# yisol/IDM-VTON

Measured on AMD Instinct MI355X. Metric: try-on images/sec at 768x1024, 30 DDIM steps, guidance 2.0, higher is better.
Workload: dtype bf16; 1 GPU; BASELINE.json configs[1]: 768x1024, 30 steps, batch 2/GPU, guidance 2.0, bf16 storage / fp32 accumulate, scheduler ddim, hipGraph on, GarmentNet batched over 6 timesteps, GarmentNet(block b+1)||TryonNet(block b) two-stream overlap on; images_per_call=2, parallelism=dp1 (image shards, one start-up RCCL weight broadcast), rccl_ranks=1

## Files before the change

### idm-vton_amd/csrc/elementwise.hip

```cpp
#include "common.cuh"
#include <string.h>

static thread_local char g_err[512] = "";
int idmvton_set_error(int code, const char* fmt, ...) {
    va_list ap; va_start(ap, fmt); vsnprintf(g_err, sizeof(g_err), fmt, ap); va_end(ap);
    return code;
}
extern "C" const char* idmvton_last_error(void) { return g_err; }
extern "C" int idmvton_abi_version(void) { return 9; }

template <typename T>
__global__ void pack_input_kernel(const idmvton_pack_input_args a) {
    const int idx = blockIdx.x * blockDim.x + threadIdx.x;
    const int total = 2 * a.B * a.hw;
    if (idx >= total) return;
    const int b2 = idx / a.hw, pix = idx - b2 * a.hw;
    const int b = b2 % a.B;
    T* o = (T*)a.out + (size_t)idx * a.cpad;
    const T* cond = (const T*)a.cond + (size_t)idx * 9;
#pragma unroll
    for (int c = 0; c < 4; ++c) o[c] = (T)a.latents[((size_t)b * 4 + c) * a.hw + pix];
#pragma unroll
    for (int c = 0; c < 9; ++c) o[4 + c] = cond[c];
    for (int c = 13; c < a.cpad; ++c) o[c] = (T)0.f;
}
extern "C" int idmvton_pack_input(const idmvton_pack_input_args* a, void* stream) {
    CHECK_ARG(a && a->latents && a->cond && a->out, IDMVTON_E_ARG, "pack_input: null pointer");
    CHECK_ARG(a->dtype == IDMVTON_F16 || a->dtype == IDMVTON_BF16, IDMVTON_E_DTYPE, "pack_input: dtype %d", a->dtype);
    CHECK_ARG(a->B > 0 && a->hw > 0 && a->cpad >= 13, IDMVTON_E_SHAPE, "pack_input: B=%d hw=%d cpad=%d", a->B, a->hw, a->cpad);
    const int total = 2 * a->B * a->hw;
    const dim3 grid((total + 255) / 256), block(256);
    if (a->dtype == IDMVTON_BF16) hipLaunchKernelGGL((pack_input_kernel<bf16_t>), grid, block, 0, (hipStream_t)stream, *a);
    else hipLaunchKernelGGL((pack_input_kernel<f16_t>), grid, block, 0, (hipStream_t)stream, *a);
    CHECK_LAUNCH("pack_input");
    return IDMVTON_OK;
}

template <typename T>
__global__ void cfg_step_kernel(const idmvton_cfg_step_args a) {
    const int idx = blockIdx.x * blockDim.x + threadIdx.x;
    if (idx >= a.B * a.hw) return;
    const int b = idx / a.hw, pix = idx - b * a.hw;
    const float c_x = a.coef[0], c_eps = a.coef[1], sigma = a.coef[2], g = a.coef[3];
    const T* eu = (const T*)a.eps_nhwc + ((size_t)b * a.hw + pix) * a.ldc;
    const T* ec = (const T*)a.eps_nhwc + ((size_t)(a.B + b) * a.hw + pix) * a.ldc;
#pragma unroll
    for (int c = 0; c < 4; ++c) {
        const size_t o = ((size_t)b * 4 + c) * a.hw + pix;
        const float u = (float)eu[c], t = (float)ec[c];
        const float eps = u + g * (t - u);
        float x = c_x * a.latents[o] + c_eps * eps;
        if (a.noise) x += sigma * a.noise[o];
        a.latents[o] = x;
    }
}
extern "C" int idmvton_cfg_step(const idmvton_cfg_step_args* a, void* stream) {
    CHECK_ARG(a && a->eps_nhwc && a->latents && a->coef, IDMVTON_E_ARG, "cfg_step: null pointer");
    CHECK_ARG(a->dtype == IDMVTON_F16 || a->dtype == IDMVTON_BF16, IDMVTON_E_DTYPE, "cfg_step: dtype %d", a->dtype);
    CHECK_ARG(a->B > 0 && a->hw > 0 && a->ldc >= 4, IDMVTON_E_SHAPE, "cfg_step: B=%d hw=%d ldc=%d", a->B, a->hw, a->ldc);
    const dim3 grid((a->B * a->hw + 255) / 256), block(256);
    if (a->dtype == IDMVTON_BF16) hipLaunchKernelGGL((cfg_step_kernel<bf16_t>), grid, block, 0, (hipStream_t)stream, *a);
    else hipLaunchKernelGGL((cfg_step_kernel<f16_t>), grid, block, 0, (hipStream_t)stream, *a);
    CHECK_LAUNCH("cfg_step");
    return IDMVTON_OK;
}

template <typename T>
__global__ void layout_kernel(const idmvton_layout_args a) {
    const size_t idx = (size_t)blockIdx.x * blockDim.x + threadIdx.x;
    if (idx >= (size_t)a.B * a.HW) return;
    const int b = (int)(idx / a.HW), pix = (int)(idx - (size_t)b * a.HW);
    if (a.to_nhwc) {
        const float* s = (const float*)a.src;
        if (a.flags & IDMVTON_LAYOUT_SPLIT) {
            T* d = (T*)a.dst + idx * 2 * a.cpad;
            for (int c = 0; c < a.C; ++c) {
                const float f = s[((size_t)b * a.C + c) * a.HW + pix] * a.scale + a.shift;
                const T hi = (T)f;
                d[c] = hi; d[a.cpad + c] = (T)(f - (float)hi);
            }
            for (int c = a.C; c < a.cpad; ++c) { d[c] = (T)0.f; d[a.cpad + c] = (T)0.f; }
            return;
        }
        T* d = (T*)a.dst + idx * a.cpad;
        for (int c = 0; c < a.C; ++c) d[c] = (T)(s[((size_t)b * a.C + c) * a.HW + pix] * a.scale + a.shift);
        for (int c = a.C; c < a.cpad; ++c) d[c] = (T)0.f;
    } else {
        float* d = (float*)a.dst;
        if (a.flags & IDMVTON_LAYOUT_NHWC_F32) {
            const float* s = (const float*)a.src + idx * a.cpad;
            for (int c = 0; c < a.C; ++c) d[((size_t)b * a.C + c) * a.HW + pix] = s[c] * a.scale + a.shift;
            return;
        }
        const T* s = (const T*)a.src + idx * a.cpad;
        for (int c = 0; c < a.C; ++c) d[((size_t)b * a.C + c) * a.HW + pix] = (float)s[c] * a.scale + a.shift;
    }
}
extern "C" int idmvton_layout(const idmvton_layout_args* a, void* stream) {
    CHECK_ARG(a && a->src && a->dst, IDMVTON_E_ARG, "layout: null pointer");
    CHECK_ARG(a->dtype == IDMVTON_F16 || a->dtype == IDMVTON_BF16, IDMVTON_E_DTYPE, "layout: dtype %d", a->dtype);
    CHECK_ARG(a->B > 0 && a->C > 0 && a->HW > 0 && a->cpad >= a->C, IDMVTON_E_SHAPE, "layout: B=%d C=%d HW=%d cpad=%d", a->B, a->C, a->HW, a->cpad);
    CHECK_ARG((a->flags & ~3) == 0 && !((a->flags & IDMVTON_LAYOUT_SPLIT) && !a->to_nhwc) && !((a->flags & IDMVTON_LAYOUT_NHWC_F32) && a->to_nhwc),
              IDMVTON_E_ARG, "layout: flags=%d (SPLIT goes with to_nhwc, NHWC_F32 with the reverse)", a->flags);
    const size_t total = (size_t)a->B * a->HW;
    const dim3 grid((unsigned)((total + 255) / 256)), block(256);
    if (a->dtype == IDMVTON_BF16) hipLaunchKernelGGL((layout_kernel<bf16_t>), grid, block, 0, (hipStream_t)stream, *a);
    else hipLaunchKernelGGL((layout_kernel<f16_t>), grid, block, 0, (hipStream_t)stream, *a);
    CHECK_LAUNCH("layout");
    return IDMVTON_OK;
}

template <typename T>
__global__ __launch_bounds__(256) void split_rows_kernel(const idmvton_split_args a) {
    typedef typename VT<T>::v8 v8;
    const int nchunk = a.cols >> 3;
    const size_t idx = (size_t)blockIdx.x * 256 + threadIdx.x;
    if (idx >= (size_t)a.rows * nchunk) return;
    const int row = (int)(idx / nchunk), c = (int)(idx - (size_t)row * nchunk) * 8;
    const float4* p = (const float4*)(a.src + (size_t)row * a.lds + c);
    const float4 t0 = p[0], t1 = p[1];
    const float v[8] = {t0.x, t0.y, t0.z, t0.w, t1.x, t1.y, t1.z, t1.w};
    v8 hi, lo;
#pragma unroll
    for (int j = 0; j < 8; ++j) { hi[j] = (T)v[j]; lo[j] = (T)(v[j] - (float)hi[j]); }
    T* d = (T*)a.dst + (size_t)row * a.ldd + c;
    *(v8*)d = hi;
    if (a.mode == IDMVTON_SPLIT_ACT) *(v8*)(d + a.cols) = lo;
    else { *(v8*)(d + a.cols) = hi; *(v8*)(d + 2 * a.cols) = lo; }
}
template <typename T>
__global__ __launch_bounds__(256) void split_t_kernel(const idmvton_split_args a) {
    typedef typename VT<T>::v8 v8;
    __shared__ float tile[64][65];
    const int r0 = blockIdx.y * 64, c0 = blockIdx.x * 64;
    for (int i = threadIdx.x; i < 64 * 64; i += 256) {
        const int r = i >> 6, c = i & 63;
        tile[r][c] = (r0 + r < a.rows && c0 + c < a.cols) ? a.src[(size_t)(r0 + r) * a.lds + c0 + c] : 0.f;
    }
    __syncthreads();
    for (int i = threadIdx.x; i < 64 * 8; i += 256) {
        const int c = i >> 3, rc = (i & 7) * 8;
        if (c0 + c >= a.cols || r0 + rc >= a.rows) continue;
        v8 hi, lo;
#pragma unroll
        for (int j = 0; j < 8; ++j) { const float f = tile[rc + j][c]; hi[j] = (T)f; lo[j] = (T)(f - (float)hi[j]); }
        T* d = (T*)a.dst + (size_t)(c0 + c) * a.ldd + r0 + rc;
        *(v8*)d = hi; *(v8*)(d + a.rows) = hi; *(v8*)(d + 2 * a.rows) = lo;
    }
}
extern "C" int idmvton_split(const idmvton_split_args* a, void* stream) {
    CHECK_ARG(a && a->src && a->dst, IDMVTON_E_ARG, "split: null pointer");
    CHECK_ARG(a->dtype == IDMVTON_F16 || a->dtype == IDMVTON_BF16, IDMVTON_E_DTYPE, "split: dtype %d", a->dtype);
    CHECK_ARG(a->mode >= IDMVTON_SPLIT_ACT && a->mode <= IDMVTON_SPLIT_W3T, IDMVTON_E_ARG, "split: mode %d", a->mode);
    CHECK_ARG(a->rows > 0 && a->cols > 0 && a->lds >= a->cols, IDMVTON_E_SHAPE, "split: rows=%d cols=%d lds=%d", a->rows, a->cols, a->lds);
    CHECK_ARG(((uintptr_t)a->dst & 15) == 0 && a->ldd % 8 == 0, IDMVTON_E_ALIGN, "split: dst alignment / ldd=%d", a->ldd);
    hipStream_t st = (hipStream_t)stream;
    if (a->mode == IDMVTON_SPLIT_W3T) {
        CHECK_ARG(a->rows % 8 == 0 && a->ldd >= 3 * a->rows, IDMVTON_E_SHAPE, "split: W3T needs rows %% 8 == 0 and ldd >= 3 rows (rows=%d ldd=%d)", a->rows, a->ldd);
        const dim3 grid((a->cols + 63) / 64, (a->rows + 63) / 64), block(256);
        if (a->dtype == IDMVTON_BF16) hipLaunchKernelGGL((split_t_kernel<bf16_t>), grid, block, 0, st, *a);
        else hipLaunchKernelGGL((split_t_kernel<f16_t>), grid, block, 0, st, *a);
    } else {
        const int k = a->mode == IDMVTON_SPLIT_ACT ? 2 : 3;
        CHECK_ARG(a->cols % 8 == 0 && a->lds % 4 == 0 && ((uintptr_t)a->src & 15) == 0 && a->ldd >= k * a->cols, IDMVTON_E_SHAPE,
                  "split: cols=%d lds=%d ldd=%d (cols %% 8 == 0, lds %% 4 == 0, ldd >= %d cols)", a->cols, a->lds, a->ldd, k);
        const size_t total = (size_t)a->rows * (a->cols >> 3);
        const dim3 grid((unsigned)((total + 255) / 256)), block(256);
        if (a->dtype == IDMVTON_BF16) hipLaunchKernelGGL((split_rows_kernel<bf16_t>), grid, block, 0, st, *a);
        else hipLaunchKernelGGL((split_rows_kernel<f16_t>), grid, block, 0, st, *a);
    }
    CHECK_LAUNCH("split");
    return IDMVTON_OK;
}

template <typename T>
__global__ void vae_sample_kernel(const idmvton_vae_sample_args a) {
    const int idx = blockIdx.x * blockDim.x + threadIdx.x;
    if (idx >= a.B * a.hw) return;
    const int b = idx / a.hw, pix = idx - b * a.hw;
    const T* m = (const T*)a.moments + (size_t)idx * a.ldm;
#pragma unroll
    for (int c = 0; c < 4; ++c) {
        const size_t o = ((size_t)b * 4 + c) * a.hw + pix;
        const float mean = (float)m[c];
        const float lv = fminf(fmaxf((float)m[4 + c], -30.f), 20.f);
        a.z[o] = (mean + __expf(0.5f * lv) * a.noise[o]) * a.scale;
    }
}
extern "C" int idmvton_vae_sample(const idmvton_vae_sample_args* a, void* stream) {
    CHECK_ARG(a && a->moments && a->noise && a->z, IDMVTON_E_ARG, "vae_sample: null pointer");
    CHECK_ARG(a->dtype == IDMVTON_F16 || a->dtype == IDMVTON_BF16, IDMVTON_E_DTYPE, "vae_sample: dtype %d", a->dtype);
    CHECK_ARG(a->B > 0 && a->hw > 0 && a->ldm >= 8, IDMVTON_E_SHAPE, "vae_sample: B=%d hw=%d ldm=%d", a->B, a->hw, a->ldm);
    const dim3 grid((a->B * a->hw + 255) / 256), block(256);
    if (a->dtype == IDMVTON_BF16) hipLaunchKernelGGL((vae_sample_kernel<bf16_t>), grid, block, 0, (hipStream_t)stream, *a);
    else hipLaunchKernelGGL((vae_sample_kernel<f16_t>), grid, block, 0, (hipStream_t)stream, *a);
    CHECK_LAUNCH("vae_sample");
    return IDMVTON_OK;
}

typedef __attribute__((ext_vector_type(8))) int i32x8;
__global__ void probe_mfma_kernel(int which, const void* a, const void* b, float* c) {
    const int lane = threadIdx.x;
    f32x16 acc;
#pragma unroll
    for (int r = 0; r < 16; ++r) acc[r] = 0.f;
    if (which == 0) acc = VT<bf16_t>::mfma(((const bf16x8*)a)[lane], ((const bf16x8*)b)[lane], acc);
    else if (which == 2) acc = __builtin_amdgcn_mfma_scale_f32_32x32x64_f8f6f4(((const i32x8*)a)[lane], ((const i32x8*)b)[lane], acc, 0, 0, 0, 0x7f7f7f7f, 0, 0x7f7f7f7f);
    else if (which == 3) acc = __builtin_amdgcn_mfma_scale_f32_32x32x64_f8f6f4(((const i32x8*)a)[lane], ((const i32x8*)b)[lane], acc, 0, 0, 0, 0x7c7c7c7c, 0, (int)0x80808080);
    else acc = VT<f16_t>::mfma(((const f16x8*)a)[lane], ((const f16x8*)b)[lane], acc);
#pragma unroll
    for (int r = 0; r < 16; ++r) c[lane * 16 + r] = acc[r];
}
extern "C" int idmvton_probe_mfma(int which, const void* a, const void* b, float* c, void* stream) {
    CHECK_ARG(a && b && c && which >= 0 && which <= 3, IDMVTON_E_ARG, "probe_mfma: bad args");
    hipLaunchKernelGGL(probe_mfma_kernel, dim3(1), dim3(64), 0, (hipStream_t)stream, which, a, b, c);
    CHECK_LAUNCH("probe_mfma");
    return IDMVTON_OK;
}

extern "C" int idmvton_sizeof(const char* name) {
#define SZ(n) if (!strcmp(name, #n)) return (int)sizeof(n);
    SZ(idmvton_seg) SZ(idmvton_gemm_conv_args) SZ(idmvton_attn_args) SZ(idmvton_layernorm_args)
    SZ(idmvton_groupnorm_args) SZ(idmvton_pack_input_args) SZ(idmvton_cfg_step_args) SZ(idmvton_layout_args)
    SZ(idmvton_vae_sample_args) SZ(idmvton_softmax_args) SZ(idmvton_attn_small_args) SZ(idmvton_attn_f8_args) SZ(idmvton_quant_f8_args) SZ(idmvton_split_args) SZ(idmvton_xattn)
#undef SZ
    return -1;
}
```

### idm-vton_amd/csrc/gemm_body.cuh

```cuda
#pragma once
#include <type_traits>
#if !defined(__gfx950__) && !defined(__gfx942__) && defined(__HIP_DEVICE_COMPILE__)
#error "gemm_body.cuh: the counted vmcnt pipeline is written for gfx94x/gfx950 (stores counted in vmcnt)"
#endif
#include "common.cuh"
#include "gemm_common.cuh"

template <typename T, int BN, int BM, int WN, int WM, int ST, bool V1, bool LIN, bool PF, bool TR, bool XA = false>
__device__ __forceinline__ void gemm_body(const GemmParams& p, char* smem, const int m0, const int n0) {
    typedef typename VT<T>::v8 v8;
    typedef typename VT<T>::v4 v4;
    constexpr int NW = WN * WM;
    constexpr int SN = BN / WN, SM = BM / WM;
    constexpr int NI = SN / 32, MI = SM / 32;
    constexpr int WBYTES = BN * 128, XBYTES = BM * 128;
    constexpr int PW_ = BN / 8, PX_ = BM / 8;
    constexpr bool UNEVEN = (PW_ % NW != 0) || (PX_ % NW != 0);
    constexpr int WI = (PW_ + NW - 1) / NW, XI = (PX_ + NW - 1) / NW;
    static_assert(BN % 8 == 0 && BM % 8 == 0 && WN * SN == BN && WM * SM == BM && NI * 32 == SN && MI * 32 == SM, "tile / wave-count mismatch");
    static_assert(!UNEVEN || (V1 && ST == 2), "round-robin piece assignment needs the two-stage ring");
    char* sW = smem;
    char* sX = smem + ST * WBYTES;

    const int lane = threadIdx.x & 63;
    const int wave = uniform(threadIdx.x >> 6);
    const int wn = wave / WM, wm = wave % WM;
    const int u = lane >> 5, l31 = lane & 31;

    const int lrow = lane >> 3, lslot = lane & 7;
    auto wj = [&](int i) { return UNEVEN ? wave + i * NW : wave * WI + i; };
    auto xj = [&](int i) { return UNEVEN ? wave + i * NW : wave * XI + i; };
    uint32_t w_off[WI];
#pragma unroll
    for (int i = 0; i < WI; ++i) {
        const int R = wj(i) * 8 + lrow;
        const int c = lslot ^ ((R >> 1) & 7);
        w_off[i] = ((uint32_t)(n0 + R) * (uint32_t)p.Ktot + c * 8) * 2u;
    }
    int x_pix[XI], x_oy[XI], x_ox[XI], x_c8[XI];
    uint32_t x_off[XI];
    const int HoWo = p.Ho * p.Wo;
    auto kbyte = [&](int t) -> uint32_t { return (uint32_t)t * 128u; };
#pragma unroll
    for (int i = 0; i < XI; ++i) {
        const int R = xj(i) * 8 + lrow;
        const int m = m0 + R;
        x_c8[i] = (lslot ^ ((R >> 1) & 7)) * 8;
        if constexpr (LIN) {
            x_off[i] = m < p.M ? ((uint32_t)m * (uint32_t)p.seg[0].pitch + p.seg[0].coff + x_c8[i]) * 2u : OOB_SENTINEL;
        } else if (m < p.M) {
            const int b = m / HoWo, rem = m - b * HoWo;
            const int oy = rem / p.Wo, ox = rem - oy * p.Wo;
            x_pix[i] = b * p.Hi * p.Wi; x_oy[i] = oy * p.stride; x_ox[i] = ox * p.stride;
        } else {
            x_pix[i] = 0; x_oy[i] = -(1 << 28); x_ox[i] = 0;
        }
    }
    const __amdgpu_buffer_rsrc_t rs_w = make_rsrc(p.w, p.w_bytes);
    const __amdgpu_buffer_rsrc_t rs_x0 = make_rsrc(p.seg[0].ptr, p.seg[0].bytes);
    const int hin = p.ups ? p.Ho : p.Hi, win = p.ups ? p.Wo : p.Wi;

    int si = 0, kseg = 0;
    auto issue = [&](int t, int buf) {
        char* dW = sW + buf * WBYTES;
        char* dX = sX + buf * XBYTES;
#pragma unroll
        for (int i = 0; i < WI; ++i) {
            if (UNEVEN && wj(i) >= PW_) continue;
            dma16(rs_w, dW + wj(i) * 1024, w_off[i] + kbyte(t));
        }
        if constexpr (LIN) {
#pragma unroll
            for (int i = 0; i < XI; ++i) {
                if (UNEVEN && xj(i) >= PX_) continue;
                dma16(rs_x0, dX + xj(i) * 1024, x_off[i] + kbyte(t));
            }
        } else {
            const idmvton_seg sg = p.seg[si];
            const __amdgpu_buffer_rsrc_t rs_x = make_rsrc(sg.ptr, sg.bytes);
#pragma unroll
            for (int i = 0; i < XI; ++i) {
                if (UNEVEN && xj(i) >= PX_) continue;
                int iy = x_oy[i] + sg.dy, ix = x_ox[i] + sg.dx;
                const bool ok = (unsigned)iy < (unsigned)hin && (unsigned)ix < (unsigned)win;
                if (p.ups) { iy >>= 1; ix >>= 1; }
                const uint32_t off = ((uint32_t)(x_pix[i] + iy * p.Wi + ix) * (uint32_t)sg.pitch + sg.coff + kseg + x_c8[i]) * 2u;
                dma16(rs_x, dX + xj(i) * 1024, ok ? off : OOB_SENTINEL);
            }
            kseg += 64;
            if (kseg >= sg.len) { kseg = 0; ++si; }
        }
    };

    idmvton_seg sgc = p.seg[0];
    __amdgpu_buffer_rsrc_t rs_xc = rs_x0;
    auto issue_part = [&](int t, int buf, int s) {
        constexpr int LPT_ = WI + XI;
        char* dW = sW + buf * WBYTES;
        char* dX = sX + buf * XBYTES;
        if constexpr (!LIN) {
            if (s == 0) { sgc = p.seg[si]; rs_xc = make_rsrc(sgc.ptr, sgc.bytes); }
        }
#pragma unroll
        for (int j = 0; j < LPT_; ++j) {
            if ((j & 3) != s) continue;
            if (j < WI) {
                if (UNEVEN && wj(j) >= PW_) continue;
                dma16(rs_w, dW + wj(j) * 1024, w_off[j] + kbyte(t));
            } else {
                const int i = j - WI;
                if (UNEVEN && xj(i) >= PX_) continue;
                if constexpr (LIN) dma16(rs_x0, dX + xj(i) * 1024, x_off[i] + kbyte(t));
                else {
                    int iy = x_oy[i] + sgc.dy, ix = x_ox[i] + sgc.dx;
                    const bool ok = (unsigned)iy < (unsigned)hin && (unsigned)ix < (unsigned)win;
                    if (p.ups) { iy >>= 1; ix >>= 1; }
                    const uint32_t off = ((uint32_t)(x_pix[i] + iy * p.Wi + ix) * (uint32_t)sgc.pitch + sgc.coff + kseg + x_c8[i]) * 2u;
                    dma16(rs_xc, dX + xj(i) * 1024, ok ? off : OOB_SENTINEL);
                }
            }
        }
        if constexpr (!LIN) {
            if (s == 3) { kseg += 64; if (kseg >= sgc.len) { kseg = 0; ++si; } }
        }
    };

    int a_row[NI], a_swz[NI], b_row[MI], b_swz[MI];
#pragma unroll
    for (int ni = 0; ni < NI; ++ni) { const int r = wn * SN + ni * 32 + l31; a_row[ni] = r * 128; a_swz[ni] = (r >> 1) & 7; }
#pragma unroll
    for (int mi = 0; mi < MI; ++mi) { const int r = wm * SM + mi * 32 + l31; b_row[mi] = r * 128; b_swz[mi] = (r >> 1) & 7; }

    f32x16 acc[NI][MI];
#pragma unroll
    for (int ni = 0; ni < NI; ++ni)
#pragma unroll
        for (int mi = 0; mi < MI; ++mi)
#pragma unroll
            for (int r = 0; r < 16; ++r) acc[ni][mi][r] = 0.f;

    auto frag_a = [&](const char* bW, int s, int ni) { return *(const v8*)(bW + a_row[ni] + (((2 * s + u) ^ a_swz[ni]) << 4)); };
    auto frag_b = [&](const char* bX, int s, int mi) { return *(const v8*)(bX + b_row[mi] + (((2 * s + u) ^ b_swz[mi]) << 4)); };
    auto compute = [&](int buf, bool spread = false, int t_next = 0, int buf_next = 0) {
        const char* bW = sW + buf * WBYTES;
        const char* bX = sX + buf * XBYTES;
        if constexpr (!PF) {
#pragma unroll
            for (int s = 0; s < 4; ++s) {
                v8 a[NI], b[MI];
#pragma unroll
                for (int ni = 0; ni < NI; ++ni) a[ni] = frag_a(bW, s, ni);
#pragma unroll
                for (int mi = 0; mi < MI; ++mi) b[mi] = frag_b(bX, s, mi);
                if constexpr (V1) {
                    if (spread) issue_part(t_next, buf_next, s);
                    __builtin_amdgcn_sched_barrier(0);
                }
#pragma unroll
                for (int ni = 0; ni < NI; ++ni)
#pragma unroll
                    for (int mi = 0; mi < MI; ++mi)
                        acc[ni][mi] = TR ? VT<T>::mfma(b[mi], a[ni], acc[ni][mi]) : VT<T>::mfma(a[ni], b[mi], acc[ni][mi]);
            }
        } else {
            v8 a[2][NI], b[2][MI];
#pragma unroll
            for (int ni = 0; ni < NI; ++ni) a[0][ni] = frag_a(bW, 0, ni);
#pragma unroll
            for (int mi = 0; mi < MI; ++mi) b[0][mi] = frag_b(bX, 0, mi);
#pragma unroll
            for (int s = 0; s < 4; ++s) {
                if (s < 3) {
#pragma unroll
                    for (int ni = 0; ni < NI; ++ni) a[(s + 1) & 1][ni] = frag_a(bW, s + 1, ni);
#pragma unroll
                    for (int mi = 0; mi < MI; ++mi) b[(s + 1) & 1][mi] = frag_b(bX, s + 1, mi);
                }
                if (spread) issue_part(t_next, buf_next, s);
                __builtin_amdgcn_sched_barrier(0);
#pragma unroll
                for (int ni = 0; ni < NI; ++ni)
#pragma unroll
                    for (int mi = 0; mi < MI; ++mi)
                        acc[ni][mi] = TR ? VT<T>::mfma(b[s & 1][mi], a[s & 1][ni], acc[ni][mi])
                                         : VT<T>::mfma(a[s & 1][ni], b[s & 1][mi], acc[ni][mi]);
                __builtin_amdgcn_sched_barrier(0);
            }
        }
    };

    v8 xkf[XA ? XA_NK : 1];
    int xa_b = 0, xa_h = 0;
    if constexpr (XA) {
        static_assert(NI == 2 && !TR, "fused cross-attention: one 64-channel head per wave");
        const int mw = m0 + wm * SM;
        xa_b = (mw < p.M ? mw : p.M - 1) / p.xa.tokens;
        xa_h = (n0 + wn * SN) >> 6;
        xattn_load_k<T>(p.xa, xa_b, xa_h, lane, xkf);
    }
    const int nt = p.Ktot >> 6;
    if constexpr (!V1) {
        issue(0, 0);
        for (int t = 0; t < nt; ++t) {
            asm volatile("s_waitcnt vmcnt(0)" ::: "memory");
            __syncthreads();
            if (t + 1 < nt) issue(t + 1, (t + 1) & 1);
            compute(t & 1);
        }
    } else {
        constexpr int LPT = WI + XI;
        static_assert((ST - 2) * LPT < 64, "vmcnt immediate is 6 bits");
#pragma unroll
        for (int s = 0; s < ST - 1; ++s)
            if (s < nt) issue(s, s);
        int cbuf = 0, ibuf = ST - 1;
        for (int t = 0; t < nt; ++t) {
            if (t + ST - 2 < nt) wait_vmcnt<(ST - 2) * LPT>(); else wait_vmcnt<0>();
            __builtin_amdgcn_s_barrier();
            asm volatile("" ::: "memory");
            compute(cbuf, t + ST - 1 < nt, t + ST - 1, ibuf);
            cbuf = cbuf + 1 == ST ? 0 : cbuf + 1;
            ibuf = ibuf + 1 == ST ? 0 : ibuf + 1;
        }
    }

    if constexpr (XA) {
        v8 xvf[XA_NV];
        xattn_load_v<T>(p.xa, xa_b, xa_h, lane, xvf);
        xattn_compute<T, MI>(p.xa, p.M, acc, m0 + wm * SM, lane, xkf, xvf);
    }
    gemm_epilogue<T, NI, MI, SN, SM, TR>(p, acc, m0, n0, wn, wm, lane);
}

template <typename T, int BN, int BM, int WN, int WM, int ST, bool V1, bool LIN, int OCC, bool PFX = false>
__global__ __launch_bounds__(WN * WM * 64, OCC) void gemm_conv_kernel(const GemmParams p) {
    __shared__ __attribute__((aligned(1024))) char smem[ST * (BN + BM) * 128];
    const int wg = xcd_remap(blockIdx.x, p.tiles_m * p.tiles_n);
    int tm, tn;
    if constexpr (!V1) { tm = wg / p.tiles_n; tn = wg - tm * p.tiles_n; }
    else {
        const int GM = p.gm > 0 ? p.gm : 1024 / BM;
        const int width = GM * p.tiles_n;
        const int grp = wg / width, rem = wg - grp * width;
        const int first = grp * GM;
        const int gsz = p.tiles_m - first < GM ? p.tiles_m - first : GM;
        tn = rem / gsz; tm = first + (rem - tn * gsz);
    }
    const int m0 = tm * BM, n0 = tn * BN;
    if constexpr (BN == 320) {
        gemm_body<T, BN, BM, WN, WM, ST, V1, LIN, OCC == 1 || PFX, false>(p, smem, m0, n0);
    } else {
        if (p.vt != nullptr && n0 >= p.vt_n0) gemm_body<T, BN, BM, WN, WM, ST, V1, LIN, OCC == 1 || PFX, true>(p, smem, m0, n0);
        else gemm_body<T, BN, BM, WN, WM, ST, V1, LIN, OCC == 1 || PFX, false>(p, smem, m0, n0);
    }
}

template <typename T, int BN, int BM, int WN, int WM, int ST, int OCC>
__global__ __launch_bounds__(WN * WM * 64, OCC) void gemm_xattn_kernel(const GemmParams p) {
    __shared__ __attribute__((aligned(1024))) char smem[ST * (BN + BM) * 128];
    const int wg = xcd_remap(blockIdx.x, p.tiles_m * p.tiles_n);
    const int GM = p.gm > 0 ? p.gm : 1024 / BM;
    const int width = GM * p.tiles_n;
    const int grp = wg / width, rem = wg - grp * width;
    const int first = grp * GM;
    const int gsz = p.tiles_m - first < GM ? p.tiles_m - first : GM;
    const int tn = rem / gsz, tm = first + (rem - tn * gsz);
    gemm_body<T, BN, BM, WN, WM, ST, true, true, OCC == 1, false, true>(p, smem, tm * BM, tn * BN);
}

template <typename T, int BN, int BM, int WN, int WM, int ST, bool V1, int OCC, bool PFX = false>
static void launch_cfg(const GemmParams& p0, bool lin, hipStream_t st) {
    GemmParams p = p0;
    p.gm = V1 ? idmvton_choose_gm(p.tiles_m, p.tiles_n, BM, BN, p.Ktot) : 0;
    const dim3 grid(p.tiles_n * p.tiles_m), block(WN * WM * 64);
    if constexpr (V1) {
        if (lin) { hipLaunchKernelGGL((gemm_conv_kernel<T, BN, BM, WN, WM, ST, true, true, OCC, PFX>), grid, block, 0, st, p); return; }
    }
    hipLaunchKernelGGL((gemm_conv_kernel<T, BN, BM, WN, WM, ST, V1, false, OCC, PFX>), grid, block, 0, st, p);
}


int gemm_tiles_v0(const GemmParams& p, bool bf16, int bn, int bm, bool lin, hipStream_t st);
int gemm_tiles_v1(const GemmParams& p, bool bf16, int bn, int bm, bool lin, hipStream_t st);
int gemm_tiles_v2(const GemmParams& p, bool bf16, int bn, int bm, bool lin, hipStream_t st);
int gemm_tiles_w8(const GemmParams& p, bool bf16, int bn, int bm, int form, bool lin, hipStream_t st);
int gemm_tiles_xattn(const GemmParams& p, bool bf16, int bn, int bm, int w8, hipStream_t st);
int launch_gemm_lin(const GemmParams& p, bool bf16, int bm, int form, int grid_cap, hipStream_t st);
```

### idm-vton_amd/csrc/gemm_common.cuh

```cuda
#pragma once
#include "common.cuh"
#include "xattn.cuh"

struct GemmParams {
    const void* w; uint32_t w_bytes; int N; int Ktot;
    int nseg; idmvton_seg seg[IDMVTON_MAX_SEG];
    int M, Ho, Wo, Hi, Wi, stride, ups;
    void* out; int ldo;
    const void* bias; const void* rowbias; int rowbias_ld; int rows_per_group;
    const void* res; int ldr;
    int mode;
    void* vt; int vt_n0; int vt_tokens; int vt_perm;
    int colscale_n; float colscale;
    int tiles_m, tiles_n;
    int gm;
    int wide;
    int res32, out32;
    int bias32;
    int out8; float o8_scale, vt8_scale;
    XAttnParams xa;
};

int idmvton_choose_gm(int tiles_m, int tiles_n, int bm, int bn, int K);

template <int N> __device__ __forceinline__ void wait_vmcnt() { asm volatile("s_waitcnt vmcnt(%0)" ::"n"(N) : "memory"); }

__device__ __forceinline__ void swap_cols8(const f32x16& c, const int gp, float (&v)[8]) {
#pragma unroll
    for (int j = 0; j < 4; ++j) {
        const auto r = __builtin_amdgcn_permlane32_swap(__float_as_uint(c[8 * gp + j]), __float_as_uint(c[8 * gp + 4 + j]), false, false);
        v[j] = __uint_as_float(r[0]);
        v[4 + j] = __uint_as_float(r[1]);
    }
}

template <typename T, int NI, int MI, int SN, int SM, bool TR>
__device__ __forceinline__ void gemm_epilogue(const GemmParams& p, f32x16 (&acc)[NI][MI], const int m0, const int n0, const int wn, const int wm,
                                              const int lane) {
    typedef typename VT<T>::v4 v4;
    typedef typename VT<T>::v8 v8;
    const int u = lane >> 5, l31 = lane & 31;
    const T* bias = (const T*)p.bias;
    if constexpr (TR) {
        if (p.out8) {
            uint8_t* vt = (uint8_t*)p.vt;
            const int Cv = p.N - p.vt_n0;
#pragma unroll
            for (int ni = 0; ni < NI; ++ni) {
                const int n = n0 + wn * SN + ni * 32 + l31;
                if (n >= p.N) continue;
                const float bv = bias ? (float)bias[n] : 0.f;
#pragma unroll
                for (int mi = 0; mi < MI; ++mi) {
                    const int m = m0 + wm * SM + mi * 32;
                    if (m >= p.M) continue;
                    const int b = m / p.vt_tokens;
                    const int tok = m - b * p.vt_tokens;
                    int4 o;
                    int w[4];
#pragma unroll
                    for (int g = 0; g < 4; ++g)
                        w[g] = pack4_fp8(clamp448((acc[ni][mi][4 * g] + bv) * p.vt8_scale), clamp448((acc[ni][mi][4 * g + 1] + bv) * p.vt8_scale),
                                         clamp448((acc[ni][mi][4 * g + 2] + bv) * p.vt8_scale), clamp448((acc[ni][mi][4 * g + 3] + bv) * p.vt8_scale));
                    o.x = w[0]; o.y = w[1]; o.z = w[2]; o.w = w[3];
                    *(int4*)(vt + ((size_t)(b * Cv + n - p.vt_n0) * p.vt_tokens + (tok & ~63) + 32 * u + ((tok >> 1) & 16))) = o;
                }
            }
            return;
        }
        if (p.vt_perm) {
            T* vt = (T*)p.vt;
            const int Cv = p.N - p.vt_n0;
#pragma unroll
            for (int ni = 0; ni < NI; ++ni) {
                const int n = n0 + wn * SN + ni * 32 + l31;
                if (n >= p.N) continue;
                const float bv = bias ? (float)bias[n] : 0.f;
#pragma unroll
                for (int mi = 0; mi < MI; ++mi)
#pragma unroll
                    for (int gp = 0; gp < 2; ++gp) {
                        const int m = m0 + wm * SM + mi * 32 + 16 * gp;
                        if (m >= p.M) continue;
                        const int b = m / p.vt_tokens;
                        const int tok = m - b * p.vt_tokens + 8 * u;
                        v8 o;
#pragma unroll
                        for (int j = 0; j < 8; ++j) o[j] = (T)(acc[ni][mi][8 * gp + j] + bv);
                        *(v8*)(vt + ((size_t)(b * Cv + n - p.vt_n0) * p.vt_tokens + tok)) = o;
                    }
            }
            return;
        }
        T* vt = (T*)p.vt;
        const int Cv = p.N - p.vt_n0;
#pragma unroll
        for (int ni = 0; ni < NI; ++ni) {
            const int n = n0 + wn * SN + ni * 32 + l31;
            if (n >= p.N) continue;
            const float bv = bias ? (float)bias[n] : 0.f;
#pragma unroll
            for (int mi = 0; mi < MI; ++mi)
#pragma unroll
                for (int g = 0; g < 4; ++g) {
                    const int m = m0 + wm * SM + mi * 32 + 8 * g + 4 * u;
                    if (m >= p.M) continue;
                    const int b = m / p.vt_tokens;
                    int tok = m - b * p.vt_tokens;
                    if (p.vt_perm) tok = (tok & ~12) | ((tok & 4) << 1) | ((tok & 8) >> 1);
                    v4 o;
#pragma unroll
                    for (int j = 0; j < 4; ++j) o[j] = (T)(acc[ni][mi][4 * g + j] + bv);
                    *(v4*)(vt + ((size_t)(b * Cv + n - p.vt_n0) * p.vt_tokens + tok)) = o;
                }
        }
        return;
    }
    T* out = (T*)p.out;
    const T* res = (const T*)p.res;
    const T* rowbias = (const T*)p.rowbias;
    if (p.wide) {
#pragma unroll
        for (int mi = 0; mi < MI; ++mi) {
            const int m = m0 + wm * SM + mi * 32 + l31;
            if (m >= p.M) continue;
            const T* rb = rowbias ? rowbias + (size_t)(m / p.rows_per_group) * p.rowbias_ld : nullptr;
            if (p.mode == IDMVTON_EPI_GEGLU) {
                if constexpr (NI % 2 == 0) {
#pragma unroll
                    for (int pr = 0; pr < NI / 2; ++pr)
#pragma unroll
                        for (int gp = 0; gp < 2; ++gp) {
                            float h[8], gt[8];
                            swap_cols8(acc[2 * pr][mi], gp, h);
                            swap_cols8(acc[2 * pr + 1][mi], gp, gt);
                            const int nh = n0 + wn * SN + pr * 64 + 16 * gp + 8 * u;
                            if (nh + 32 >= p.N) continue;
                            const int jo = ((n0 + wn * SN + pr * 64) >> 1) + 16 * gp + 8 * u;
                            if (bias) {
                                const v8 bh = *(const v8*)(bias + nh), bg = *(const v8*)(bias + nh + 32);
#pragma unroll
                                for (int j = 0; j < 8; ++j) { h[j] += (float)bh[j]; gt[j] += (float)bg[j]; }
                            }
                            v8 o;
#pragma unroll
                            for (int j = 0; j < 8; ++j) o[j] = (T)(h[j] * gelu_erf(gt[j]));
                            *(v8*)(out + (size_t)m * p.ldo + jo) = o;
                        }
                }
                continue;
            }
#pragma unroll
            for (int ni = 0; ni < NI; ++ni) {
#pragma unroll
                for (int gp = 0; gp < 2; ++gp) {
                    float v[8];
                    swap_cols8(acc[ni][mi], gp, v);
                    const int n = n0 + wn * SN + ni * 32 + 16 * gp + 8 * u;
                    if (n >= p.N) continue;
                    if (bias) {
                        if (p.bias32) {
                            const float4* bp = (const float4*)((const float*)p.bias + n);
                            const float4 b0 = bp[0], b1 = bp[1];
                            v[0] += b0.x; v[1] += b0.y; v[2] += b0.z; v[3] += b0.w;
                            v[4] += b1.x; v[5] += b1.y; v[6] += b1.z; v[7] += b1.w;
                        } else {
                            const v8 bb = *(const v8*)(bias + n);
#pragma unroll
                            for (int j = 0; j < 8; ++j) v[j] += (float)bb[j];
                        }
                    }
                    if (rb) {
                        const v8 bb = *(const v8*)(rb + n);
#pragma unroll
                        for (int j = 0; j < 8; ++j) v[j] += (float)bb[j];
                    }
                    if (n < p.colscale_n) {
#pragma unroll
                        for (int j = 0; j < 8; ++j) v[j] *= p.colscale;
                    }
                    if constexpr (NI * MI <= 8)
                    if (p.out8) {
                        int2 o;
                        o.x = pack4_fp8(clamp448(v[0] * p.o8_scale), clamp448(v[1] * p.o8_scale), clamp448(v[2] * p.o8_scale), clamp448(v[3] * p.o8_scale));
                        o.y = pack4_fp8(clamp448(v[4] * p.o8_scale), clamp448(v[5] * p.o8_scale), clamp448(v[6] * p.o8_scale), clamp448(v[7] * p.o8_scale));
                        *(int2*)((uint8_t*)p.out + (size_t)m * p.ldo + n) = o;
                        continue;
                    }
                    if (p.mode == IDMVTON_EPI_GELU) {
#pragma unroll
                        for (int j = 0; j < 8; ++j) v[j] = gelu_erf(v[j]);
                    } else if (p.mode == IDMVTON_EPI_QUICKGELU) {
#pragma unroll
                        for (int j = 0; j < 8; ++j) v[j] = v[j] / (1.0f + __expf(-1.702f * v[j]));
                    }
                    if (res) {
                        if (p.res32) {
                            const float4* rp = (const float4*)((const float*)p.res + (size_t)m * p.ldr + n);
                            const float4 r0 = rp[0], r1 = rp[1];
                            v[0] += r0.x; v[1] += r0.y; v[2] += r0.z; v[3] += r0.w;
                            v[4] += r1.x; v[5] += r1.y; v[6] += r1.z; v[7] += r1.w;
                        } else {
                            const v8 rr = *(const v8*)(res + (size_t)m * p.ldr + n);
#pragma unroll
                            for (int j = 0; j < 8; ++j) v[j] += (float)rr[j];
                        }
                    }
                    if (p.out32) {
                        float4* op = (float4*)((float*)p.out + (size_t)m * p.ldo + n);
                        op[0] = make_float4(v[0], v[1], v[2], v[3]);
                        op[1] = make_float4(v[4], v[5], v[6], v[7]);
                    } else {
                        v8 o;
#pragma unroll
                        for (int j = 0; j < 8; ++j) o[j] = (T)v[j];
                        *(v8*)(out + (size_t)m * p.ldo + n) = o;
                    }
                }
            }
        }
        return;
    }
    if constexpr (NI * MI <= 8)
#pragma unroll
    for (int mi = 0; mi < MI; ++mi) {
        const int m = m0 + wm * SM + mi * 32 + l31;
        if (m >= p.M) continue;
        const T* rb = rowbias ? rowbias + (size_t)(m / p.rows_per_group) * p.rowbias_ld : nullptr;
        if (p.mode == IDMVTON_EPI_GEGLU) {
            if constexpr (NI % 2 == 0) {
#pragma unroll
                for (int pr = 0; pr < NI / 2; ++pr)
#pragma unroll
                    for (int g = 0; g < 4; ++g) {
                        const int nh = n0 + wn * SN + pr * 64 + 8 * g + 4 * u;
                        if (nh + 32 >= p.N) continue;
                        const int jo = ((n0 + wn * SN + pr * 64) >> 1) + 8 * g + 4 * u;
                        v4 o;
#pragma unroll
                        for (int j = 0; j < 4; ++j) {
                            float h = acc[2 * pr][mi][4 * g + j], gt = acc[2 * pr + 1][mi][4 * g + j];
                            if (bias) { h += (float)bias[nh + j]; gt += (float)bias[nh + 32 + j]; }
                            o[j] = (T)(h * gelu_erf(gt));
                        }
                        *(v4*)(out + (size_t)m * p.ldo + jo) = o;
                    }
            }
            continue;
        }
#pragma unroll
        for (int ni = 0; ni < NI; ++ni)
#pragma unroll
            for (int g = 0; g < 4; ++g) {
                const int n = n0 + wn * SN + ni * 32 + 8 * g + 4 * u;
                if (n >= p.N) continue;
                float v[4];
#pragma unroll
                for (int j = 0; j < 4; ++j) v[j] = acc[ni][mi][4 * g + j];
                if (bias) {
                    const v4 bb = *(const v4*)(bias + n);
#pragma unroll
                    for (int j = 0; j < 4; ++j) v[j] += (float)bb[j];
                }
                if (rb) {
                    const v4 bb = *(const v4*)(rb + n);
#pragma unroll
                    for (int j = 0; j < 4; ++j) v[j] += (float)bb[j];
                }
                if (n < p.colscale_n) {
#pragma unroll
                    for (int j = 0; j < 4; ++j) v[j] *= p.colscale;
                }
                if (p.mode == IDMVTON_EPI_GELU) {
#pragma unroll
                    for (int j = 0; j < 4; ++j) v[j] = gelu_erf(v[j]);
                } else if (p.mode == IDMVTON_EPI_QUICKGELU) {
#pragma unroll
                    for (int j = 0; j < 4; ++j) v[j] = v[j] / (1.0f + __expf(-1.702f * v[j]));
                }
                if (res) {
                    const v4 rr = *(const v4*)(res + (size_t)m * p.ldr + n);
#pragma unroll
                    for (int j = 0; j < 4; ++j) v[j] += (float)rr[j];
                }
                v4 o;
#pragma unroll
                for (int j = 0; j < 4; ++j) o[j] = (T)v[j];
                *(v4*)(out + (size_t)m * p.ldo + n) = o;
            }
    }
}
```

### idm-vton_amd/csrc/gemm_conv.hip

```cpp
#include <cstdlib>
#include <cstring>
#include <vector>
#include "gemm_body.cuh"

int launch_gemm_lin(const GemmParams& p, bool bf16, int bm, int form, int grid_cap, hipStream_t st);

#include <map>
#include <mutex>
#include <tuple>
int idmvton_choose_gm(int tiles_m, int tiles_n, int bm, int bn, int K) {
    static const char* env = getenv("IDMVTON_GM");
    if (env) return atoi(env);
    static const bool model = getenv("IDMVTON_GM_MODEL") && atoi(getenv("IDMVTON_GM_MODEL")) != 0;
    if (!model) return 0;
    static std::mutex mu;
    static std::map<std::tuple<int, int, int, int, int>, int> cache;
    const auto key = std::make_tuple(tiles_m, tiles_n, bm, bn, K);
    std::lock_guard<std::mutex> lk(mu);
    auto it = cache.find(key);
    if (it != cache.end()) return it->second;
    const int T = tiles_m * tiles_n, q = T / 8, r = T % 8;
    static const long cap = getenv("IDMVTON_GM_CAP_KB") ? atol(getenv("IDMVTON_GM_CAP_KB")) << 10 : (2l << 20);
    long best = -1; int best_gm = 0;
    for (int gm = 1; gm <= tiles_m; ++gm) {
        if (gm > 1 && (long)gm * bm * K * 2 > cap) break;
        long cost = 0;
        for (int x = 0; x < 8; ++x) {
            const int lo = x < r ? x * (q + 1) : r * (q + 1) + (x - r) * q, n = x < r ? q + 1 : q;
            int m_lo = tiles_m, m_hi = -1;
            std::vector<char> ms(tiles_m, 0), ns(tiles_n, 0);
            int cm = 0, cn = 0;
            for (int wg = lo; wg < lo + n; ++wg) {
                const int width = gm * tiles_n, grp = wg / width, rem = wg - grp * width, first = grp * gm;
                const int gsz = tiles_m - first < gm ? tiles_m - first : gm;
                const int tn = rem / gsz, tm = first + (rem - tn * gsz);
                if (!ms[tm]) { ms[tm] = 1; ++cm; }
                if (!ns[tn]) { ns[tn] = 1; ++cn; }
            }
            (void)m_lo; (void)m_hi;
            cost += (long)cm * bm + (long)cn * bn;
        }
        if (best < 0 || cost < best) { best = cost; best_gm = gm; }
    }
    cache[key] = best_gm;
    return best_gm;
}

static int launch_gemm(const GemmParams& p0, bool bf16, int variant, int bn, int bm, bool lin, hipStream_t st) {
    GemmParams p = p0;
    int form = 0;
    int grid_cap = 0;
    if (variant == 5) { form = bm & 15; grid_cap = (bm & 0x4000) ? 5 : 0; bm &= ~(15 | 0x4000); }
    p.tiles_n = (p.N + bn - 1) / bn;
    p.tiles_m = (p.M + bm - 1) / bm;
    int rc = 1;
    if (p.mode == IDMVTON_EPI_XATTN) {
        if (bm != 64 && p.xa.tokens % 64 != 0) {
            bm = 64;
            p.tiles_m = (p.M + bm - 1) / bm;
        }
        if (gemm_tiles_xattn(p, bf16, bn, bm, variant == 6 && bn == 128 && bm == 128, st))
            return idmvton_set_error(IDMVTON_E_ARG, "gemm_conv: IDMVTON_EPI_XATTN runs on the 128x64, 128x128 and 128x256 tiles (got %dx%d)", bn, bm);
        CHECK_LAUNCH("gemm_conv");
        return IDMVTON_OK;
    }
    if (variant == 0) rc = gemm_tiles_v0(p, bf16, bn, bm, lin, st);
    else if (variant == 1) rc = gemm_tiles_v1(p, bf16, bn, bm, lin, st);
    else if (variant == 2) rc = gemm_tiles_v2(p, bf16, bn, bm, lin, st);
    else if (variant == 5) {
        if (!(bn == 256 && (bm == 256 || bm == 192))) return idmvton_set_error(IDMVTON_E_ARG, "gemm_conv: variant 5 is the 256x256 / 256x192 tile");
        if (lin) rc = launch_gemm_lin(p, bf16, bm, form, grid_cap, st);
        else if (bm == 256) rc = gemm_tiles_v1(p, bf16, 256, 256, lin, st);
        else {
            p.tiles_n = (p.N + 127) / 128; p.tiles_m = (p.M + 255) / 256;
            rc = gemm_tiles_v1(p, bf16, 128, 256, lin, st);
        }
    } else if (variant == 6) {
        const int form6 = bm & 15;
        bm &= ~15;
        p.tiles_m = (p.M + bm - 1) / bm;
        if (bn == 320 && (p.vt || !p.wide || p.out8 || p.mode == IDMVTON_EPI_GEGLU)) {
            const int fbn = bn == 320 ? 128 : bn, fbm = bn == 320 ? 256 : bm;
            p.tiles_n = (p.N + fbn - 1) / fbn;
            p.tiles_m = (p.M + fbm - 1) / fbm;
            rc = gemm_tiles_v1(p, bf16, fbn, fbm, lin, st);
        } else rc = gemm_tiles_w8(p, bf16, bn, bm, form6, lin, st);
    } else return idmvton_set_error(IDMVTON_E_ARG, "gemm_conv: unknown variant %d", variant);
    if (rc) return idmvton_set_error(IDMVTON_E_ARG, "gemm_conv: variant %d has no %dx%d tile", variant, bn, bm);
    CHECK_LAUNCH("gemm_conv");
    return IDMVTON_OK;
}

extern "C" int idmvton_gemm_conv(const idmvton_gemm_conv_args* a, void* stream) {
    CHECK_ARG(a != nullptr, IDMVTON_E_ARG, "gemm_conv: null args");
    CHECK_ARG(a->dtype == IDMVTON_F16 || a->dtype == IDMVTON_BF16, IDMVTON_E_DTYPE, "gemm_conv: dtype %d", a->dtype);
    CHECK_ARG(a->M > 0 && a->N > 0 && a->Ktot > 0, IDMVTON_E_SHAPE, "gemm_conv: M=%d N=%d K=%d", a->M, a->N, a->Ktot);
    CHECK_ARG(a->Ktot % 64 == 0, IDMVTON_E_SHAPE, "gemm_conv: Ktot=%d must be a multiple of 64", a->Ktot);
    CHECK_ARG(a->N % 4 == 0, IDMVTON_E_SHAPE, "gemm_conv: N=%d must be a multiple of 4", a->N);
    CHECK_ARG(a->nseg >= 1 && a->nseg <= IDMVTON_MAX_SEG, IDMVTON_E_SHAPE, "gemm_conv: nseg=%d", a->nseg);
    int ksum = 0;
    for (int s = 0; s < a->nseg; ++s) {
        const idmvton_seg& g = a->seg[s];
        CHECK_ARG(g.ptr && g.len > 0 && g.len % 64 == 0, IDMVTON_E_SHAPE, "gemm_conv: seg %d len=%d", s, g.len);
        CHECK_ARG(g.pitch % 8 == 0 && g.coff % 8 == 0, IDMVTON_E_ALIGN, "gemm_conv: seg %d pitch=%d coff=%d", s, g.pitch, g.coff);
        CHECK_ARG(g.bytes < 0x80000000u, IDMVTON_E_SHAPE, "gemm_conv: seg %d tensor >= 2 GiB", s);
        CHECK_ARG(((uintptr_t)g.ptr & 15) == 0, IDMVTON_E_ALIGN, "gemm_conv: seg %d pointer not 16-byte aligned", s);
        ksum += g.len;
    }
    CHECK_ARG(ksum == a->Ktot, IDMVTON_E_SHAPE, "gemm_conv: segment lengths sum to %d, Ktot=%d", ksum, a->Ktot);
    CHECK_ARG(a->Ho > 0 && a->Wo > 0 && a->Hi > 0 && a->Wi > 0 && a->stride > 0 && a->M % (a->Ho * a->Wo) == 0,
              IDMVTON_E_SHAPE, "gemm_conv: geometry M=%d Ho=%d Wo=%d", a->M, a->Ho, a->Wo);
    if (a->ups) CHECK_ARG(a->stride == 1 && a->Ho <= 2 * a->Hi && a->Ho >= 2 * a->Hi - 1 && a->Wo <= 2 * a->Wi && a->Wo >= 2 * a->Wi - 1, IDMVTON_E_SHAPE,
                          "gemm_conv: ups=1 needs stride 1 and an output grid of 2Hi x 2Wi or one short of it (Ho=%d Hi=%d Wo=%d Wi=%d)", a->Ho, a->Hi, a->Wo, a->Wi);
    CHECK_ARG(a->w && ((uintptr_t)a->w & 15) == 0, IDMVTON_E_ALIGN, "gemm_conv: weight pointer");
    const uint64_t wbytes = (uint64_t)a->N * a->Ktot * 2;
    CHECK_ARG(wbytes + (uint64_t)128 * a->Ktot * 2 < 0xFFFFFFFFull, IDMVTON_E_SHAPE, "gemm_conv: weight too large");
    const bool geglu = a->mode == IDMVTON_EPI_GEGLU, xattn = a->mode == IDMVTON_EPI_XATTN;
    CHECK_ARG(a->mode == IDMVTON_EPI_NONE || a->mode == IDMVTON_EPI_GELU || a->mode == IDMVTON_EPI_QUICKGELU || geglu || xattn, IDMVTON_E_ARG, "gemm_conv: mode %d", a->mode);
    CHECK_ARG(a->colscale_n >= 0 && a->colscale_n % 4 == 0 && !(geglu && a->colscale_n), IDMVTON_E_ARG, "gemm_conv: colscale_n=%d", a->colscale_n);
    if (geglu) CHECK_ARG(a->N % 64 == 0 && !a->res && !a->rowbias && !a->vt, IDMVTON_E_ARG, "gemm_conv: GEGLU needs N%%64==0, no res/rowbias/vt");
    CHECK_ARG(a->out || (a->vt && a->vt_n0 == 0), IDMVTON_E_ARG, "gemm_conv: null out");
    if (a->out) CHECK_ARG(a->ldo % 4 == 0 && ((uintptr_t)a->out & 7) == 0, IDMVTON_E_ALIGN, "gemm_conv: out alignment");
    if (a->res) CHECK_ARG(a->ldr % 4 == 0 && ((uintptr_t)a->res & 7) == 0, IDMVTON_E_ALIGN, "gemm_conv: res alignment");
    if (a->bias) CHECK_ARG(((uintptr_t)a->bias & 7) == 0, IDMVTON_E_ALIGN, "gemm_conv: bias alignment");
    if (a->rowbias) CHECK_ARG(a->rowbias_ld % 4 == 0 && a->rows_per_group > 0 && ((uintptr_t)a->rowbias & 7) == 0,
                              IDMVTON_E_ALIGN, "gemm_conv: rowbias");
    if (a->vt && a->vt_perm) CHECK_ARG(((uintptr_t)a->vt & 15) == 0, IDMVTON_E_ALIGN, "gemm_conv: vt pointer not 16-byte aligned");
    if (a->vt && a->vt_perm) CHECK_ARG(a->vt_tokens % 16 == 0, IDMVTON_E_ARG, "gemm_conv: vt_perm needs vt_tokens %% 16 == 0 (got %d)", a->vt_tokens);
    if (a->vt) CHECK_ARG(a->vt_tokens > 0 && a->vt_tokens % 4 == 0 && a->M % a->vt_tokens == 0 && a->vt_n0 % 64 == 0 &&
                         a->vt_n0 >= 0 && a->vt_n0 < a->N && ((uintptr_t)a->vt & 7) == 0,
                         IDMVTON_E_ARG, "gemm_conv: vt_tokens=%d vt_n0=%d", a->vt_tokens, a->vt_n0);

    GemmParams p;
    memset(&p.xa, 0, sizeof(p.xa));
    if (xattn) {
        const idmvton_xattn* x = a->xattn;
        CHECK_ARG(x != nullptr && (x->nseg == 1 || x->nseg == 2), IDMVTON_E_ARG, "gemm_conv: IDMVTON_EPI_XATTN needs `xattn` with 1 or 2 key segments");
        CHECK_ARG(a->N % 64 == 0 && !a->bias && !a->res && !a->rowbias && !a->vt && !a->colscale_n && !a->io_flags &&
                  a->nseg == 1 && a->Ho == 1 && a->Hi == 1 && a->Wo == a->M && a->Wi == a->M && a->out && a->ldo % 8 == 0 && ((uintptr_t)a->out & 15) == 0,
                  IDMVTON_E_ARG, "gemm_conv: IDMVTON_EPI_XATTN is a plain Linear with N %% 64 == 0 and nothing else in its epilogue");
        CHECK_ARG(x->tokens > 0 && x->tokens % 32 == 0 && a->M % x->tokens == 0, IDMVTON_E_SHAPE, "gemm_conv: xattn.tokens=%d (rows per batch element, a multiple of 32 dividing M=%d)", x->tokens, a->M);
        for (int s = 0; s < x->nseg; ++s) {
            const int nk_max = s == 0 ? 96 : 32;
            CHECK_ARG(x->k[s] && x->vt[s] && x->nk[s] > 0 && x->nk[s] <= nk_max && x->k_rows[s] >= ((x->nk[s] + 31) & ~31) && x->ldk[s] >= a->N && x->ldk[s] % 8 == 0 &&
                      x->ldvt[s] >= ((x->nk[s] + 15) & ~15) && x->ldvt[s] % 8 == 0 && (((uintptr_t)x->k[s] | (uintptr_t)x->vt[s]) & 15) == 0, IDMVTON_E_SHAPE,
                      "gemm_conv: xattn segment %d: nk=%d (<= %d) k_rows=%d (>= round32(nk)) ldk=%d ldvt=%d (>= round16(nk))", s, x->nk[s], nk_max, x->k_rows[s], x->ldk[s], x->ldvt[s]);
            p.xa.k[s] = x->k[s]; p.xa.vt[s] = x->vt[s]; p.xa.ldk[s] = x->ldk[s]; p.xa.ldvt[s] = x->ldvt[s]; p.xa.nk[s] = x->nk[s]; p.xa.krows[s] = x->k_rows[s];
        }
        p.xa.nseg = x->nseg; p.xa.tokens = x->tokens; p.xa.vchan = a->N; p.xa.ip_scale = x->ip_scale;
    } else CHECK_ARG(a->xattn == nullptr, IDMVTON_E_ARG, "gemm_conv: `xattn` without mode IDMVTON_EPI_XATTN");
    p.w = a->w; p.w_bytes = (uint32_t)wbytes; p.N = a->N; p.Ktot = a->Ktot;
    p.nseg = a->nseg;
    for (int s = 0; s < IDMVTON_MAX_SEG; ++s) p.seg[s] = a->seg[s < a->nseg ? s : a->nseg - 1];
    p.M = a->M; p.Ho = a->Ho; p.Wo = a->Wo; p.Hi = a->Hi; p.Wi = a->Wi; p.stride = a->stride; p.ups = a->ups ? 1 : 0;
    p.out = a->out; p.ldo = a->ldo; p.bias = a->bias; p.rowbias = a->rowbias; p.rowbias_ld = a->rowbias_ld;
    p.rows_per_group = a->rows_per_group > 0 ? a->rows_per_group : 1; p.res = a->res; p.ldr = a->ldr; p.mode = a->mode;
    p.vt = a->vt; p.vt_n0 = a->vt_n0; p.vt_tokens = a->vt_tokens > 0 ? a->vt_tokens : 4; p.vt_perm = a->vt_perm ? 1 : 0;
    p.colscale_n = a->colscale_n; p.colscale = a->colscale;
    p.tiles_m = p.tiles_n = 0; p.gm = 0;
    {
        auto a16 = [](const void* q) { return ((uintptr_t)q & 15) == 0; };
        const int n_out = geglu ? a->N / 2 : a->N;
        p.wide = n_out % 8 == 0 && a->N % 8 == 0 && a->colscale_n % 8 == 0 && (!a->out || (a->ldo % 8 == 0 && a16(a->out))) &&
                 (!a->res || (a->ldr % 8 == 0 && a16(a->res))) && (!a->bias || a16(a->bias)) &&
                 (!a->rowbias || (a->rowbias_ld % 8 == 0 && a16(a->rowbias))) && (!a->vt || a->vt_n0 % 8 == 0);
    }

    int variant = 1, bn = 64, bm = 64;
    static const bool env_narrow = getenv("IDMVTON_EPILOGUE_8B") != nullptr;
    if ((a->tile_hint & 0x8000) || env_narrow) p.wide = 0;
    p.res32 = (a->io_flags & IDMVTON_IO_RES_F32) ? 1 : 0;
    p.out32 = (a->io_flags & IDMVTON_IO_OUT_F32) ? 1 : 0;
    p.bias32 = (a->io_flags & IDMVTON_IO_BIAS_F32) ? 1 : 0;
    if (p.bias32) CHECK_ARG(a->bias && p.wide && !geglu && !a->vt && ((uintptr_t)a->bias & 15) == 0, IDMVTON_E_ARG,
                            "gemm_conv: IDMVTON_IO_BIAS_F32 needs a 16-byte aligned bias and the plain 16-byte epilogue (no GEGLU, no vt)");
    CHECK_ARG((a->io_flags & ~15) == 0, IDMVTON_E_ARG, "gemm_conv: io_flags=%d", a->io_flags);
    p.out8 = (a->io_flags & IDMVTON_IO_OUT_F8) ? 1 : 0;
    p.o8_scale = a->f8_out_scale; p.vt8_scale = a->f8_vt_scale;
    if (p.out8) {
        CHECK_ARG(a->io_flags == IDMVTON_IO_OUT_F8 && a->mode == IDMVTON_EPI_NONE && !a->res && !a->rowbias && p.wide,
                  IDMVTON_E_ARG, "gemm_conv: IDMVTON_IO_OUT_F8 needs the plain 16-byte epilogue (no activation / residual / rowbias / fp32 IO)");
        CHECK_ARG((!a->out || a->f8_out_scale > 0.f) && (!a->vt || (a->f8_vt_scale > 0.f && a->vt_tokens % 64 == 0 && ((uintptr_t)a->vt & 15) == 0)),
                  IDMVTON_E_ARG, "gemm_conv: IDMVTON_IO_OUT_F8: scales > 0, vt_tokens %% 64 == 0 (got %d), 16-byte aligned vt", a->vt_tokens);
    }
    if (p.res32 || p.out32) {
        CHECK_ARG((a->io_flags & ~7) == 0 && !geglu && !a->vt, IDMVTON_E_ARG, "gemm_conv: io_flags=%d (fp32 res / out: no GEGLU, no vt)", a->io_flags);
        CHECK_ARG(!p.res32 || a->res, IDMVTON_E_ARG, "gemm_conv: IDMVTON_IO_RES_F32 without res");
        CHECK_ARG(p.wide, IDMVTON_E_ALIGN, "gemm_conv: the fp32 residual stream needs the 16-byte epilogue (N, ldo, ldr multiples of 8, 16-byte aligned pointers)");
    }
    if (a->tile_hint) { variant = (a->tile_hint >> 28) & 0xf; bn = (a->tile_hint >> 16) & 0xfff; bm = a->tile_hint & 0x7fff; }
    else {
        static const int cand[5][2] = {{256, 256}, {128, 256}, {128, 128}, {128, 64}, {64, 64}};
        for (int i = 0; i < 5; ++i) {
            const int n_ = cand[i][0], m_ = cand[i][1];
            if (geglu && n_ < 128) continue;
            if (xattn && (n_ != 128)) continue;
            if (a->vt && a->vt_n0 % n_ != 0) continue;
            if (i < 4 && (n_ > ((a->N + 63) & ~63) || m_ > ((a->M + 63) & ~63))) continue;
            bn = n_; bm = m_;
            if ((long)((a->N + n_ - 1) / n_) * ((a->M + m_ - 1) / m_) >= 200) break;
        }
    }
    if (geglu) CHECK_ARG(bn >= 128, IDMVTON_E_ARG, "gemm_conv: GEGLU needs BN >= 128 (64-row wave tiles)");
    if (a->vt) CHECK_ARG(a->vt_n0 % bn == 0, IDMVTON_E_ARG, "gemm_conv: vt_n0 %% BN != 0");
    const idmvton_seg& s0 = a->seg[0];
    const bool lin = a->nseg == 1 && a->Ho == 1 && a->Hi == 1 && a->Wo == a->M && a->Wi == a->M && a->stride == 1 &&
                     !a->ups && s0.dy == 0 && s0.dx == 0 && (uint64_t)a->M * s0.pitch * 2 < 0x80000000ull;
    if (!a->tile_hint && bn == 256 && bm == 256 && lin) { variant = 5; bm = 257; }
    else if (!a->tile_hint && !xattn) {
        if (bn == 256 && bm == 256) variant = 6;
        else if (bn == 128 && bm == 128) variant = 6;
        if (a->N > 256 && a->N <= 320 && p.wide && !a->vt && !geglu && !p.out8 && (a->M + 191) / 192 >= 200) { variant = 6; bn = 320; bm = 192; }
    }
    hipStream_t st = (hipStream_t)stream;
    return launch_gemm(p, a->dtype == IDMVTON_BF16, variant, bn, bm, lin, st);
}
```

### idm-vton_amd/csrc/gemm_lin.hip

```cpp
#include "gemm_common.cuh"
#include <type_traits>

template <typename T, int BM, int WN, int WM, int DMA_SPLIT, int WAIT_AT>
__device__ __forceinline__ void gemm_lin_persistent(const GemmParams& p, char* smem) {
    typedef typename VT<T>::v8 v8;
    constexpr int BN = 256, NW = WN * WM;
    constexpr int SN = BN / WN, SM = BM / WM, NI = SN / 32, MI = SM / 32;
    constexpr int PWW = BN / (8 * NW), PWX = BM / (8 * NW);
    static_assert(PWW * 8 * NW == BN && PWX * 8 * NW == BM && NI * 32 * WN == BN && MI * 32 * WM == BM, "tile / wave-count mismatch");
    constexpr int OPW = BN * 128;
    constexpr int BUF = (BN + BM) * 128;

    const int lane = threadIdx.x & 63;
    const int wave = uniform(threadIdx.x >> 6);
    const int wn = wave / WM, wm = wave % WM;
    const int u = lane >> 5, l31 = lane & 31;

    const int ntiles = p.tiles_m * p.tiles_n, G = gridDim.x;
    auto coords = [&](int idx, int& m0, int& n0) {
        const int wg = xcd_remap(idx, ntiles);
        const int GM = p.gm > 0 ? p.gm : 1024 / BM;
        const int width = GM * p.tiles_n;
        const int grp = wg / width, rem = wg - grp * width;
        const int first = grp * GM;
        const int gsz = p.tiles_m - first < GM ? p.tiles_m - first : GM;
        const int tn = rem / gsz;
        m0 = (first + (rem - tn * gsz)) * BM;
        n0 = tn * BN;
    };

    const int lrow = lane >> 3, lslot = lane & 7;
    uint32_t w_off[PWW], x_off[PWX];
    auto set_offsets = [&](int m0, int n0) {
#pragma unroll
        for (int i = 0; i < PWW; ++i) {
            const int R = (wave * PWW + i) * 8 + lrow;
            w_off[i] = ((uint32_t)(n0 + R) * (uint32_t)p.Ktot + (lslot ^ ((R >> 1) & 7)) * 8) * 2u;
        }
#pragma unroll
        for (int i = 0; i < PWX; ++i) {
            const int R = (wave * PWX + i) * 8 + lrow;
            const int m = m0 + R;
            x_off[i] = m < p.M ? ((uint32_t)m * (uint32_t)p.seg[0].pitch + p.seg[0].coff + (lslot ^ ((R >> 1) & 7)) * 8) * 2u : OOB_SENTINEL;
        }
    };
    const __amdgpu_buffer_rsrc_t rs_w = make_rsrc(p.w, p.w_bytes);
    const __amdgpu_buffer_rsrc_t rs_x = make_rsrc(p.seg[0].ptr, p.seg[0].bytes);
    char* const dW = smem + wave * (PWW * 1024);
    char* const dX = smem + OPW + wave * (PWX * 1024);
    auto dma_w = [&](int i, int buf_off, uint32_t koff) {
        __builtin_amdgcn_raw_ptr_buffer_load_lds(rs_w, LDS_PTR(dW + buf_off + i * 1024), 16, w_off[i], koff, 0, 0);
    };
    auto dma_x = [&](int i, int buf_off, uint32_t koff) {
        __builtin_amdgcn_raw_ptr_buffer_load_lds(rs_x, LDS_PTR(dX + buf_off + i * 1024), 16, x_off[i], koff, 0, 0);
    };
    auto dma_first = [&](int buf_off) {
#pragma unroll
        for (int i = 0; i < PWW; ++i) dma_w(i, buf_off, 0u);
#pragma unroll
        for (int i = 0; i < PWX; ++i) dma_x(i, buf_off, 0u);
    };

    const int swz = (l31 >> 1) & 7;
    int fa_off[4], fb_off[4];
#pragma unroll
    for (int s = 0; s < 4; ++s) {
        const int ch = ((2 * s + u) ^ swz) << 4;
        fa_off[s] = (wn * SN + l31) * 128 + ch;
        fb_off[s] = OPW + (wm * SM + l31) * 128 + ch;
    }
    v8 fa[2][NI], fb[2][MI];
    f32x16 acc[NI][MI];

    auto read_all = [&](int set, int s, int buf_off) {
#pragma unroll
        for (int ni = 0; ni < NI; ++ni) fa[set][ni] = *(const v8*)(smem + buf_off + fa_off[s] + ni * 4096);
#pragma unroll
        for (int mi = 0; mi < MI; ++mi) fb[set][mi] = *(const v8*)(smem + buf_off + fb_off[s] + mi * 4096);
    };
    constexpr int NMF = NI * MI;
    constexpr int NRD = NI + MI;
    auto pin = [&](int nrd, int nv) {
#pragma unroll
        for (int i = 0; i < NMF; ++i) {
            __builtin_amdgcn_sched_group_barrier(0x008, 1, 0);
            if (i < nrd) __builtin_amdgcn_sched_group_barrier(0x100, 1, 0);
            if (i >= NMF - nv) __builtin_amdgcn_sched_group_barrier(0x010, 1, 0);
            if (i < nv - NMF) __builtin_amdgcn_sched_group_barrier(0x010, 1, 0);
        }
    };

    const int nt = p.Ktot >> 6;
    int idx = blockIdx.x, m0, n0, nm0 = 0, nn0 = 0;
    bool has_next = false;
    int cur = 0;

    auto run_tile = [&](auto trc) {
        constexpr bool TR = decltype(trc)::value;
        auto mfma_range = [&](int set, int i0, int i1) {
#pragma unroll
            for (int k = i0; k < i1; ++k) {
                const int ni = k / MI, mi = k % MI;
                acc[ni][mi] = TR ? VT<T>::mfma(fb[set][mi], fa[set][ni], acc[ni][mi]) : VT<T>::mfma(fa[set][ni], fb[set][mi], acc[ni][mi]);
            }
        };
#pragma unroll
        for (int ni = 0; ni < NI; ++ni)
#pragma unroll
            for (int mi = 0; mi < MI; ++mi)
#pragma unroll
                for (int r = 0; r < 16; ++r) acc[ni][mi][r] = 0.f;
        __builtin_amdgcn_s_barrier();
        asm volatile("" ::: "memory");
        read_all(0, 0, cur);
        for (int t = 0; t + 1 < nt; ++t) {
            const int nxt = cur ^ BUF;
            const uint32_t koff = (uint32_t)(t + 1) * 128u;
            read_all(1, 1, cur);
#pragma unroll
            for (int i = 0; i < PWW; ++i) dma_w(i, nxt, koff);
            if constexpr (DMA_SPLIT == 1) {
#pragma unroll
                for (int i = 0; i < PWX; ++i) dma_x(i, nxt, koff);
            }
            mfma_range(0, 0, NMF);
            pin(NRD, DMA_SPLIT == 0 ? PWW : PWW + PWX);
            __builtin_amdgcn_sched_barrier(0);
            read_all(0, 2, cur);
            if constexpr (DMA_SPLIT == 0) {
#pragma unroll
                for (int i = 0; i < PWX; ++i) dma_x(i, nxt, koff);
            }
            mfma_range(1, 0, NMF);
            pin(NRD, DMA_SPLIT == 0 ? PWX : 0);
            __builtin_amdgcn_sched_barrier(0);
            read_all(1, 3, cur);
            mfma_range(0, 0, NMF);
            pin(NRD, 0);
            __builtin_amdgcn_sched_barrier(0);
            mfma_range(1, 0, WAIT_AT);
            __builtin_amdgcn_sched_barrier(0);
            asm volatile("s_waitcnt vmcnt(0) lgkmcnt(0)" ::: "memory");
            __builtin_amdgcn_s_barrier();
            asm volatile("" ::: "memory");
            __builtin_amdgcn_sched_barrier(0);
            read_all(0, 0, nxt);
            mfma_range(1, WAIT_AT, NMF);
#pragma unroll
            for (int i = 0; i < NMF - WAIT_AT; ++i) {
                __builtin_amdgcn_sched_group_barrier(0x008, 1, 0);
                if (i < NRD) __builtin_amdgcn_sched_group_barrier(0x100, 1, 0);
                if (i == NMF - WAIT_AT - 1 && NRD > NMF - WAIT_AT) __builtin_amdgcn_sched_group_barrier(0x100, NRD - (NMF - WAIT_AT), 0);
            }
            __builtin_amdgcn_sched_barrier(0);
            cur = nxt;
        }
        if (has_next) {
            set_offsets(nm0, nn0);
            dma_first(cur ^ BUF);
        }
        read_all(1, 1, cur);
        mfma_range(0, 0, NMF);
        pin(NRD, 0);
        __builtin_amdgcn_sched_barrier(0);
        read_all(0, 2, cur);
        mfma_range(1, 0, NMF);
        pin(NRD, 0);
        __builtin_amdgcn_sched_barrier(0);
        read_all(1, 3, cur);
        mfma_range(0, 0, NMF);
        pin(NRD, 0);
        __builtin_amdgcn_sched_barrier(0);
        mfma_range(1, 0, NMF);
        if (has_next) asm volatile("s_waitcnt vmcnt(0)" ::: "memory");
        gemm_epilogue<T, NI, MI, SN, SM, TR>(p, acc, m0, n0, wn, wm, lane);
    };

    coords(idx, m0, n0);
    set_offsets(m0, n0);
    dma_first(0);
    asm volatile("s_waitcnt vmcnt(0)" ::: "memory");
    for (;;) {
        const int nidx = idx + G;
        has_next = nidx < ntiles;
        if (has_next) coords(nidx, nm0, nn0);
        if (p.vt != nullptr && n0 >= p.vt_n0) run_tile(std::true_type{});
        else run_tile(std::false_type{});
        if (!has_next) break;
        cur ^= BUF; idx = nidx; m0 = nm0; n0 = nn0;
    }
}

template <typename T, int BM, int WN, int WM, int DMA_SPLIT, int WAIT_AT>
__global__ __launch_bounds__(512, 2) void gemm_lin_kernel(const GemmParams p) {
    __shared__ __attribute__((aligned(1024))) char smem[2 * (256 + BM) * 128];
    gemm_lin_persistent<T, BM, WN, WM, DMA_SPLIT, WAIT_AT>(p, smem);
}

static int persistent_grid(int ntiles, int grid_cap) {
    static int cus = 0;
    if (!cus) {
        int dev = 0, n = 0;
        if (hipGetDevice(&dev) != hipSuccess || hipDeviceGetAttribute(&n, hipDeviceAttributeMultiprocessorCount, dev) != hipSuccess || n < 8) n = 256;
        cus = n & ~7;
    }
    const int cap = grid_cap > 0 ? grid_cap : cus;
    return ntiles < cap ? ntiles : cap;
}
template <typename T>
static int launch_lin(const GemmParams& p0, int bm, int form, int grid_cap, hipStream_t st) {
    GemmParams p = p0;
    p.gm = idmvton_choose_gm(p.tiles_m, p.tiles_n, bm, 256, p.Ktot);
    const dim3 grid(persistent_grid(p.tiles_n * p.tiles_m, grid_cap)), block(512);
    if (bm == 192) hipLaunchKernelGGL((gemm_lin_kernel<T, 192, 4, 2, 0, 2>), grid, block, 0, st, p);
    else if (form == 0) hipLaunchKernelGGL((gemm_lin_kernel<T, 256, 2, 4, 0, 2>), grid, block, 0, st, p);
    else hipLaunchKernelGGL((gemm_lin_kernel<T, 256, 2, 4, 1, 2>), grid, block, 0, st, p);
    return 0;
}
int launch_gemm_lin(const GemmParams& p, bool bf16, int bm, int form, int grid_cap, hipStream_t st) {
    return bf16 ? launch_lin<bf16_t>(p, bm, form, grid_cap, st) : launch_lin<f16_t>(p, bm, form, grid_cap, st);
}
```

### idm-vton_amd/csrc/gemm_tiles_xattn.hip

```cpp
#include "gemm_body.cuh"

template <typename T>
static int run(const GemmParams& p0, int bn, int bm, int w8, hipStream_t st) {
    GemmParams p = p0;
    p.gm = idmvton_choose_gm(p.tiles_m, p.tiles_n, bm, bn, p.Ktot);
    const dim3 grid(p.tiles_n * p.tiles_m);
    if (bn == 128 && bm == 128 && w8) hipLaunchKernelGGL((gemm_xattn_kernel<T, 128, 128, 2, 4, 3, 2>), grid, dim3(512), 0, st, p);
    else if (bn == 128 && bm == 64) hipLaunchKernelGGL((gemm_xattn_kernel<T, 128, 64, 2, 2, 3, 2>), grid, dim3(256), 0, st, p);
    else if (bn == 128 && bm == 128) hipLaunchKernelGGL((gemm_xattn_kernel<T, 128, 128, 2, 2, 3, 1>), grid, dim3(256), 0, st, p);
    else if (bn == 128 && bm == 256) hipLaunchKernelGGL((gemm_xattn_kernel<T, 128, 256, 2, 4, 3, 2>), grid, dim3(512), 0, st, p);
    else return 1;
    return 0;
}
int gemm_tiles_xattn(const GemmParams& p, bool bf16, int bn, int bm, int w8, hipStream_t st) {
    return bf16 ? run<bf16_t>(p, bn, bm, w8, st) : run<f16_t>(p, bn, bm, w8, st);
}
```

### idm-vton_amd/ffi.py

```python
import ctypes as C
import os

_HERE = os.path.dirname(os.path.abspath(__file__))
LIB_PATH = os.environ.get("IDMVTON_HIP_LIB") or os.path.join(_HERE, "libidmvton_hip.so")

F16, BF16, F32, F8E4M3 = 0, 1, 2, 3
EPI_NONE, EPI_GEGLU, EPI_GELU, EPI_QUICKGELU, EPI_XATTN = 0, 1, 2, 3, 4
ATTN_SELF, ATTN_CROSS = 0, 1
IO_RES_F32, IO_OUT_F32, IO_BIAS_F32, IO_OUT_F8 = 1, 2, 4, 8
GN_X_F32, GN_Y_SPLIT, GN_AFFINE_F32 = 1, 2, 4
LAYOUT_SPLIT, LAYOUT_NHWC_F32 = 1, 2
SPLIT_ACT, SPLIT_W3, SPLIT_W3T = 0, 1, 2
MAX_SEG = 24
ABI_VERSION = 9

i32, u32, f32, vp = C.c_int32, C.c_uint32, C.c_float, C.c_void_p


class Seg(C.Structure):
    _fields_ = [("ptr", vp), ("bytes", u32), ("pitch", i32), ("coff", i32), ("len", i32), ("dy", i32), ("dx", i32)]


class XAttn(C.Structure):
    _fields_ = [("nseg", i32), ("k", vp * 2), ("ldk", i32 * 2), ("k_rows", i32 * 2), ("vt", vp * 2), ("ldvt", i32 * 2), ("nk", i32 * 2),
                ("tokens", i32), ("ip_scale", f32)]


class GemmConvArgs(C.Structure):
    _fields_ = [("dtype", i32), ("w", vp), ("N", i32), ("Ktot", i32), ("nseg", i32), ("seg", Seg * MAX_SEG),
                ("M", i32), ("Ho", i32), ("Wo", i32), ("Hi", i32), ("Wi", i32), ("stride", i32), ("ups", i32),
                ("out", vp), ("ldo", i32), ("bias", vp), ("rowbias", vp), ("rowbias_ld", i32),
                ("rows_per_group", i32), ("res", vp), ("ldr", i32), ("mode", i32), ("vt", vp), ("vt_n0", i32),
                ("vt_tokens", i32), ("tile_hint", i32), ("vt_perm", i32), ("io_flags", i32), ("xattn", C.POINTER(XAttn)),
                ("colscale_n", i32), ("colscale", f32), ("f8_out_scale", f32), ("f8_vt_scale", f32)]


class AttnArgs(C.Structure):
    _fields_ = [("dtype", i32), ("mode", i32), ("B", i32), ("heads", i32), ("Nq", i32), ("q", vp), ("ldq", i32),
                ("out", vp), ("ldo", i32), ("nseg", i32), ("k", vp * 2), ("ldk", i32 * 2), ("vt", vp * 2),
                ("ldvt", i32 * 2), ("nk", i32 * 2), ("k_rows", i32 * 2), ("seg_b0", i32 * 2), ("ip_scale", f32), ("tune", i32), ("q_prescaled", i32)]


class LayerNormArgs(C.Structure):
    _fields_ = [("dtype", i32), ("rows", i32), ("C", i32), ("x", vp), ("ldx", i32), ("gamma", vp), ("beta", vp),
                ("eps", f32), ("y", vp), ("ldy", i32), ("y2", vp), ("ldy2", i32), ("x_f32", i32)]


class GroupNormArgs(C.Structure):
    _fields_ = [("dtype", i32), ("B", i32), ("HW", i32), ("C", i32), ("groups", i32), ("x", vp), ("C1", i32),
                ("x2", vp), ("gamma", vp), ("beta", vp), ("eps", f32), ("silu", i32), ("y", vp), ("stats", vp), ("stats_doubles", i32),
                ("flags", i32)]


class PackInputArgs(C.Structure):
    _fields_ = [("dtype", i32), ("B", i32), ("hw", i32), ("cpad", i32), ("latents", vp), ("cond", vp), ("out", vp)]


class CfgStepArgs(C.Structure):
    _fields_ = [("dtype", i32), ("B", i32), ("hw", i32), ("ldc", i32), ("eps_nhwc", vp), ("latents", vp),
                ("noise", vp), ("coef", vp)]


class LayoutArgs(C.Structure):
    _fields_ = [("dtype", i32), ("B", i32), ("C", i32), ("HW", i32), ("cpad", i32), ("to_nhwc", i32), ("src", vp),
                ("dst", vp), ("scale", f32), ("shift", f32), ("flags", i32)]


class VaeSampleArgs(C.Structure):
    _fields_ = [("dtype", i32), ("B", i32), ("hw", i32), ("ldm", i32), ("moments", vp), ("noise", vp), ("z", vp),
                ("scale", f32)]


class AttnSmallArgs(C.Structure):
    _fields_ = [("dtype", i32), ("B", i32), ("heads", i32), ("Lq", i32), ("Lk", i32), ("d", i32), ("q", vp), ("ldq", i32),
                ("k", vp), ("ldk", i32), ("v", vp), ("ldv", i32), ("out", vp), ("ldo", i32), ("scale", f32), ("causal", i32)]


class AttnF8Args(C.Structure):
    _fields_ = [("out_dtype", i32), ("B", i32), ("heads", i32), ("Nq", i32), ("q8", vp), ("ldq", i32), ("out", vp), ("ldo", i32),
                ("nseg", i32), ("k8", vp * 2), ("ldk", i32 * 2), ("vt8", vp * 2), ("ldvt", i32 * 2), ("nk", i32 * 2), ("k_rows", i32 * 2),
                ("seg_b0", i32 * 2), ("qk_scale_exp", i32), ("v_scale_exp", i32)]


class QuantF8Args(C.Structure):
    _fields_ = [("dtype", i32), ("mode", i32), ("rows", i32), ("cols", i32), ("src", vp), ("lds", i32), ("dst", vp), ("ldd", i32), ("scale", f32)]


class SoftmaxArgs(C.Structure):
    _fields_ = [("dtype", i32), ("rows", i32), ("n", i32), ("ld", i32), ("x", vp), ("scale", f32), ("y_split", vp), ("ldy", i32), ("n_valid", i32)]


class SplitArgs(C.Structure):
    _fields_ = [("dtype", i32), ("mode", i32), ("rows", i32), ("cols", i32), ("src", vp), ("lds", i32), ("dst", vp), ("ldd", i32)]


STRUCTS = {"idmvton_seg": Seg, "idmvton_gemm_conv_args": GemmConvArgs, "idmvton_attn_args": AttnArgs,
           "idmvton_layernorm_args": LayerNormArgs, "idmvton_groupnorm_args": GroupNormArgs,
           "idmvton_pack_input_args": PackInputArgs, "idmvton_cfg_step_args": CfgStepArgs,
           "idmvton_layout_args": LayoutArgs, "idmvton_vae_sample_args": VaeSampleArgs, "idmvton_softmax_args": SoftmaxArgs,
           "idmvton_attn_small_args": AttnSmallArgs, "idmvton_attn_f8_args": AttnF8Args, "idmvton_quant_f8_args": QuantF8Args,
           "idmvton_split_args": SplitArgs, "idmvton_xattn": XAttn}

SYMBOLS = ["idmvton_last_error", "idmvton_abi_version", "idmvton_sizeof", "idmvton_gemm_conv", "idmvton_attn_fwd",
           "idmvton_layernorm", "idmvton_groupnorm", "idmvton_pack_input", "idmvton_cfg_step", "idmvton_layout",
           "idmvton_vae_sample", "idmvton_softmax_rows", "idmvton_probe_mfma", "idmvton_groupnorm_stats_doubles",
           "idmvton_attn_small", "idmvton_rccl_unique_id", "idmvton_rccl_comm_init", "idmvton_rccl_bcast_arena",
           "idmvton_rccl_comm_destroy", "idmvton_attn_f8", "idmvton_quant_f8", "idmvton_split", "idmvton_attn_fwd_shared",
           "idmvton_attn_f8_shared"]

_lib = None


class HipLibraryMissing(RuntimeError):
    pass


def lib():
    global _lib
    if _lib is not None:
        return _lib
    if not os.path.exists(LIB_PATH):
        raise HipLibraryMissing(f"{LIB_PATH} not built: run `make -C {os.path.join(_HERE, 'csrc')}` "
                                "(or __graft_entry__.build()); there is no CPU fallback")
    L = C.CDLL(LIB_PATH)
    for s in SYMBOLS:
        if not hasattr(L, s):
            raise HipLibraryMissing(f"{LIB_PATH} does not export {s}")
    L.idmvton_last_error.restype = C.c_char_p
    L.idmvton_sizeof.argtypes = [C.c_char_p]
    L.idmvton_abi_version.restype = C.c_int
    v = L.idmvton_abi_version()
    if v != ABI_VERSION:
        raise HipLibraryMissing(f"{LIB_PATH} implements C ABI version {v}, this binding needs {ABI_VERSION}: rebuild it "
                                f"(`make -C {os.path.join(_HERE, 'csrc')}`)")
    for name, st in STRUCTS.items():
        n = L.idmvton_sizeof(name.encode())
        if n != C.sizeof(st):
            raise HipLibraryMissing(f"ABI drift: sizeof({name}) is {n} in the library, {C.sizeof(st)} in ffi.py")
    for s in ("idmvton_gemm_conv", "idmvton_attn_fwd", "idmvton_layernorm", "idmvton_groupnorm",
              "idmvton_pack_input", "idmvton_cfg_step", "idmvton_layout", "idmvton_vae_sample", "idmvton_softmax_rows",
              "idmvton_attn_small", "idmvton_attn_f8", "idmvton_quant_f8", "idmvton_split"):
        getattr(L, s).argtypes = [vp, vp]
        getattr(L, s).restype = C.c_int
    for s in ("idmvton_attn_fwd_shared", "idmvton_attn_f8_shared"):
        getattr(L, s).argtypes = [vp, C.POINTER(i32), vp]
        getattr(L, s).restype = C.c_int
    L.idmvton_probe_mfma.argtypes = [C.c_int, vp, vp, vp, vp]
    L.idmvton_groupnorm_stats_doubles.argtypes = [C.c_int] * 4
    L.idmvton_groupnorm_stats_doubles.restype = C.c_int
    L.idmvton_rccl_unique_id.argtypes = [vp]
    L.idmvton_rccl_comm_init.argtypes = [vp, C.c_int, C.c_int, C.POINTER(vp)]
    L.idmvton_rccl_bcast_arena.argtypes = [vp, vp, C.c_uint64, C.c_int, C.c_uint64, vp]
    L.idmvton_rccl_comm_destroy.argtypes = [vp]
    for s in ("idmvton_rccl_unique_id", "idmvton_rccl_comm_init", "idmvton_rccl_bcast_arena", "idmvton_rccl_comm_destroy"):
        getattr(L, s).restype = C.c_int
    _lib = L
    return L


def call(fn_name, args, stream):
    L = lib()
    rc = getattr(L, fn_name)(C.byref(args), C.c_void_p(stream))
    if rc != 0:
        raise RuntimeError(f"{fn_name} failed ({rc}): {L.idmvton_last_error().decode()}")


def call_shared(fn_name, args, seg_nb, stream):
    L = lib()
    nb = (i32 * 2)(*seg_nb)
    rc = getattr(L, fn_name)(C.byref(args), nb, C.c_void_p(stream))
    if rc != 0:
        raise RuntimeError(f"{fn_name} failed ({rc}): {L.idmvton_last_error().decode()}")
```

### idm-vton_amd/ops.py

```python
import ctypes as C
import json
import os

import torch

from . import ffi

_DT = {torch.float16: ffi.F16, torch.bfloat16: ffi.BF16}


def _dt(t):
    try:
        return _DT[t.dtype]
    except KeyError:
        raise TypeError(f"idm_vton_amd ops take float16/bfloat16 tensors, got {t.dtype}") from None


def _stream():
    return torch.cuda.current_stream().cuda_stream


PROFILE = None


def _call(fn_name, args, flops=0.0, bytes_=0.0, seg_nb=None):
    launch = (lambda: ffi.call(fn_name, args, _stream())) if seg_nb is None else (lambda: ffi.call_shared(fn_name, args, seg_nb, _stream()))
    if PROFILE is None:
        launch()
        return
    e0, e1 = torch.cuda.Event(enable_timing=True), torch.cuda.Event(enable_timing=True)
    e0.record()
    launch()
    e1.record()
    PROFILE.append((fn_name, e0, e1, flops, bytes_))


TUNE_PATH = os.environ.get("IDMVTON_TUNE_TABLE") or os.path.join(os.path.dirname(os.path.abspath(__file__)), "tune_gfx950.json")
_TUNE = {"gemm": {}, "attn": {}}
RECORD = None


def load_tune(path=TUNE_PATH):
    global _TUNE
    _TUNE = {"gemm": {}, "attn": {}}
    if path and os.path.exists(path):
        with open(path) as f:
            t = json.load(f)
        _TUNE = {"gemm": dict(t.get("gemm", {})), "attn": dict(t.get("attn", {}))}
        for kind in ("gemm", "attn") if os.environ.get("IDMVTON_TUNE_NO_MIRROR") != "1" else ():
            for k, v in list(_TUNE[kind].items()):
                d, rest = k.split(",", 1)
                if d in ("0", "1"):
                    _TUNE[kind].setdefault(("1" if d == "0" else "0") + "," + rest, v)
    return _TUNE


def gemm_key(a):
    return "%d,%d,%d,%d,%d,%d,%d,%d,%d,%d" % (a.dtype, a.M, a.N, a.Ktot, a.nseg, a.Wo, a.stride, a.ups, a.mode, 1 if a.vt else 0)


def attn_key(a):
    return "%d,%d,%d,%d,%d,%d,%d,%d,%d" % (a.dtype, a.mode, a.B, a.heads, a.Nq, a.nseg, a.nk[0], a.nk[1] if a.nseg > 1 else 0,
                                          a.seg_b0[1] if a.nseg > 1 else 0)


def _dev(t):
    if not t.is_cuda:
        raise RuntimeError("idm_vton_amd ops run on the GPU only (tensor is on %s); there is no CPU fallback" % t.device)
    return t


def _ptr(t):
    return None if t is None else _dev(t).data_ptr()


class SegSpec:
    __slots__ = ("t", "coff", "len", "dy", "dx")

    def __init__(self, t, coff, length, dy=0, dx=0):
        self.t, self.coff, self.len, self.dy, self.dx = t, coff, length, dy, dx


def gemm_conv(segs, w, M, *, Ho=1, Wo=None, Hi=1, Wi=None, stride=1, ups=False, out=None, ldo=None, bias=None,
              rowbias=None, rowbias_ld=0, rows_per_group=1, res=None, ldr=None, geglu=False, gelu=False, quick_gelu=False, vt=None,
              vt_n0=0, vt_tokens=0, vt_perm=True, colscale_n=0, colscale=1.0, tile_hint=0, out_f32=False, xattn=None, f8=None):
    if f8 is not None:
        if res is not None or rowbias is not None or geglu or gelu or quick_gelu or (bias is not None and bias.dtype == torch.float32):
            raise ValueError("gemm_conv(f8=...): no residual / rowbias / activation, and the bias in the storage dtype (not fp32)")
        if vt is not None and vt_tokens % 64 != 0:
            raise ValueError(f"gemm_conv(f8=...): vt_tokens must be a multiple of 64 (got {vt_tokens})")
    a = ffi.GemmConvArgs()
    a.dtype = _dt(w)
    N, Ktot = w.shape
    a.w, a.N, a.Ktot = _ptr(w), N, Ktot
    a.nseg = len(segs)
    for i, s in enumerate(segs):
        t = _dev(s.t)
        g = a.seg[i]
        pitch = t.shape[-1]
        for d in range(t.dim() - 2, -1, -1):
            if t.shape[d] > 1:
                pitch = t.stride(d)
                break
        extent = 1 + sum((n - 1) * st for n, st in zip(t.shape, t.stride()))
        g.ptr, g.bytes, g.pitch = t.data_ptr(), extent * t.element_size(), pitch
        g.coff, g.len, g.dy, g.dx = s.coff, s.len, s.dy, s.dx
    Wo = M if Wo is None else Wo
    Wi = M if Wi is None else Wi
    a.M, a.Ho, a.Wo, a.Hi, a.Wi, a.stride, a.ups = M, Ho, Wo, Hi, Wi, stride, int(bool(ups))
    n_out = N // 2 if geglu else (vt_n0 if vt is not None else N)
    if out is None and n_out > 0:
        out = torch.empty((M, n_out), dtype=torch.uint8 if f8 is not None else (torch.float32 if out_f32 else w.dtype), device=w.device)
    if f8 is not None:
        if (out is not None and out.dtype != torch.uint8) or (vt is not None and vt.dtype != torch.uint8):
            raise TypeError("gemm_conv(f8=...): out / vt must be uint8 (e4m3 bytes)")
        a.f8_out_scale, a.f8_vt_scale = float(f8[0]), float(f8[1])
    a.io_flags = ffi.IO_OUT_F8 if f8 is not None else (
        (ffi.IO_RES_F32 if res is not None and res.dtype == torch.float32 else 0) |
        (ffi.IO_OUT_F32 if out is not None and out.dtype == torch.float32 else 0) |
        (ffi.IO_BIAS_F32 if bias is not None and bias.dtype == torch.float32 else 0))
    a.out = _ptr(out)
    a.ldo = (ldo if ldo is not None else (out.stride(-2) if out is not None else 0))
    a.bias = _ptr(bias)
    a.rowbias, a.rowbias_ld, a.rows_per_group = _ptr(rowbias), rowbias_ld, rows_per_group
    a.res = _ptr(res)
    a.ldr = (ldr if ldr is not None else (res.stride(-2) if res is not None else 0))
    a.mode = ffi.EPI_GEGLU if geglu else (ffi.EPI_GELU if gelu else (ffi.EPI_QUICKGELU if quick_gelu else ffi.EPI_NONE))
    xa, xflops = None, 0.0
    if xattn is not None:
        xa = ffi.XAttn()
        xa.nseg, xa.tokens, xa.ip_scale = len(xattn["segs"]), xattn["tokens"], xattn.get("ip_scale", 1.0)
        for i, sg in enumerate(xattn["segs"]):
            xa.k[i], xa.vt[i], xa.ldk[i], xa.ldvt[i], xa.nk[i], xa.k_rows[i] = _ptr(sg["k"]), _ptr(sg["vt"]), sg["ldk"], sg["ldvt"], sg["nk"], sg["k_rows"]
            xflops += 4.0 * M * N * sg["nk"]
        a.mode, a.xattn = ffi.EPI_XATTN, C.pointer(xa)
    a.vt, a.vt_n0, a.vt_tokens = _ptr(vt), vt_n0, vt_tokens
    a.vt_perm = int(bool(vt_perm)) if vt is not None else 0
    a.colscale_n, a.colscale = colscale_n, colscale
    a.tile_hint = tile_hint if tile_hint else _TUNE["gemm"].get(gemm_key(a), 0)
    if RECORD is not None:
        RECORD.append(("gemm", gemm_key(a), type(a).from_buffer_copy(a), (segs, w, out, bias, rowbias, res, vt, xa, xattn)))
    seen, xbytes = set(), 0
    for sg in segs:
        if sg.t.data_ptr() not in seen:
            seen.add(sg.t.data_ptr())
            xbytes += sg.t.numel() * sg.t.element_size()
    esz = w.element_size()
    obytes = (M * (N // 2 if geglu else N)) * (out.element_size() if out is not None else esz) + (M * N * res.element_size() if res is not None else 0)
    _call("idmvton_gemm_conv", a, flops=2.0 * M * N * Ktot + xflops, bytes_=float(xbytes + N * Ktot * esz + obytes))
    return out


def xattn_q_weight(w):
    return w.index_select(0, key_order_index(w.shape[0], w.device)).contiguous()


def key_order_index(n, device=None):
    if n % 16:
        raise ValueError("key order needs a multiple of 16 keys, got %d" % n)
    i = torch.arange(n, device=device)
    return (i & ~12) | ((i & 4) << 1) | ((i & 8) >> 1)


def key_order(vt):
    return vt.index_select(-1, key_order_index(vt.shape[-1], vt.device)).contiguous()


def round16(n):
    return (n + 15) // 16 * 16


def linear(x, w, **kw):
    M, K = x.shape
    return gemm_conv([SegSpec(x, 0, K)], w, M, **kw)


def conv_segs(x, k, pad, coff=0, length=None):
    length = x.shape[-1] if length is None else length
    return [SegSpec(x, coff, length, ky - pad, kx - pad) for ky in range(k) for kx in range(k)]


QSCALE = 0.125 * 1.4426950408889634


def attention(q, out, segs, heads, *, mode=ffi.ATTN_SELF, ip_scale=1.0, B=None, Nq=None, ldq=None, ldo=None, tune=0, q_prescaled=False):
    a = ffi.AttnArgs()
    a.dtype, a.mode = _dt(q), mode
    a.B = q.shape[0] if B is None else B
    a.Nq = q.shape[1] if Nq is None else Nq
    a.heads = heads
    a.q, a.ldq = _ptr(q), (q.stride(-2) if ldq is None else ldq)
    a.out, a.ldo = _ptr(out), (out.stride(-2) if ldo is None else ldo)
    a.nseg = len(segs)
    for i, s in enumerate(segs):
        a.k[i], a.vt[i] = _ptr(s["k"]), _ptr(s["vt"])
        a.ldk[i], a.ldvt[i] = s["ldk"], s["ldvt"]
        a.nk[i], a.k_rows[i], a.seg_b0[i] = s["nk"], s.get("k_rows", 0), s.get("b0", 0)
    a.ip_scale = ip_scale
    a.q_prescaled = int(bool(q_prescaled))
    a.tune = tune
    if not tune:
        t = _TUNE["attn"].get(attn_key(a), 0)
        a.tune = t if (q_prescaled or ((t >> 16) & 0xff) not in (7, 8, 16)) else 0
    if RECORD is not None:
        RECORD.append(("attn", attn_key(a), type(a).from_buffer_copy(a), (q, out, segs)))
    fl = 0.0
    for s in segs:
        fl += 4.0 * (a.B - s.get("b0", 0)) * heads * a.Nq * s["nk"] * 64
    nb = _seg_nb(segs)
    _call("idmvton_attn_fwd_shared" if nb else "idmvton_attn_fwd", a, flops=fl, bytes_=2.0 * a.B * a.Nq * heads * 64 * q.element_size(), seg_nb=nb)
    return out


def _seg_nb(segs):
    nb = [int(s.get("nb", 0) or 0) for s in segs] + [0] * (2 - len(segs))
    return nb if any(nb) else None


def quant_f8(src, scale, mode=0, out=None):
    rows, cols = src.shape
    ldd = cols if mode == 0 else (cols + 63) // 64 * 64
    if out is None:
        out = torch.empty((rows, ldd), dtype=torch.uint8, device=src.device)
    a = ffi.QuantF8Args()
    a.dtype, a.mode, a.rows, a.cols = _dt(src), mode, rows, cols
    a.src, a.lds, a.dst, a.ldd, a.scale = _ptr(src), src.stride(0), _ptr(out), out.stride(0), scale
    _call("idmvton_quant_f8", a, bytes_=float(rows * cols * (src.element_size() + 1)))
    return out


def attention_f8(q8, out, segs, heads, *, qk_scale_exp, v_scale_exp, B, Nq, ldq=None, ldo=None):
    a = ffi.AttnF8Args()
    a.out_dtype, a.B, a.heads, a.Nq = _dt(out), B, heads, Nq
    a.q8, a.ldq = _ptr(q8), (q8.stride(-2) if ldq is None else ldq)
    a.out, a.ldo = _ptr(out), (out.stride(-2) if ldo is None else ldo)
    a.nseg = len(segs)
    fl = 0.0
    for i, s in enumerate(segs):
        a.k8[i], a.vt8[i] = _ptr(s["k8"]), _ptr(s["vt8"])
        a.ldk[i], a.ldvt[i] = s["ldk"], s["ldvt"]
        a.nk[i], a.k_rows[i], a.seg_b0[i] = s["nk"], s.get("k_rows", 0), s.get("b0", 0)
        fl += 4.0 * (B - s.get("b0", 0)) * heads * Nq * s["nk"] * 64
    a.qk_scale_exp, a.v_scale_exp = qk_scale_exp, v_scale_exp
    nb = _seg_nb(segs)
    _call("idmvton_attn_f8_shared" if nb else "idmvton_attn_f8", a, flops=fl, bytes_=float(B * Nq * heads * 64 * (1 + out.element_size())), seg_nb=nb)
    return out


def attention_small(q, k, v, out, heads, d, *, scale, causal=False, B=None, Lq=None, Lk=None, ldq=None, ldk=None, ldv=None, ldo=None):
    a = ffi.AttnSmallArgs()
    a.dtype = _dt(q)
    a.B = q.shape[0] if B is None else B
    a.heads, a.d = heads, d
    a.Lq = q.shape[1] if Lq is None else Lq
    a.Lk = k.shape[1] if Lk is None else Lk
    a.q, a.ldq = _ptr(q), (q.stride(-2) if ldq is None else ldq)
    a.k, a.ldk = _ptr(k), (k.stride(-2) if ldk is None else ldk)
    a.v, a.ldv = _ptr(v), (v.stride(-2) if ldv is None else ldv)
    a.out, a.ldo = _ptr(out), (out.stride(-2) if ldo is None else ldo)
    a.scale, a.causal = scale, int(bool(causal))
    _call("idmvton_attn_small", a, flops=4.0 * a.B * heads * a.Lq * a.Lk * d)
    return out


def layernorm(x, gamma, beta, eps=1e-5, out=None, out2=None):
    rows, Cc = x.shape
    if out is None:
        out = torch.empty((rows, Cc), dtype=gamma.dtype, device=x.device)
    a = ffi.LayerNormArgs()
    a.dtype, a.rows, a.C = _dt(gamma), rows, Cc
    a.x_f32 = int(x.dtype == torch.float32)
    a.x, a.ldx = _ptr(x), x.stride(0)
    a.gamma, a.beta, a.eps = _ptr(gamma), _ptr(beta), eps
    a.y, a.ldy = _ptr(out), out.stride(0)
    a.y2, a.ldy2 = _ptr(out2), (out2.stride(0) if out2 is not None else 0)
    _call("idmvton_layernorm", a, bytes_=(x.element_size() + (1.0 + (out2 is not None)) * out.element_size()) * rows * Cc)
    return out


def groupnorm(x, gamma, beta, groups, eps, silu, stats, x2=None, out=None, split_dtype=None):
    B, HW, C1 = x.shape
    Cc = C1 + (x2.shape[-1] if x2 is not None else 0)
    prec = split_dtype is not None
    if prec and not (x.dtype == gamma.dtype == beta.dtype == torch.float32 and (x2 is None or x2.dtype == torch.float32)):
        raise TypeError("groupnorm(split_dtype=...): x, gamma and beta must be float32")
    if out is None:
        out = torch.empty((B, HW, 2 * Cc if prec else Cc), dtype=split_dtype if prec else x.dtype, device=x.device)
    a = ffi.GroupNormArgs()
    a.dtype, a.B, a.HW, a.C, a.groups = _dt(out), B, HW, Cc, groups
    a.flags = (ffi.GN_X_F32 | ffi.GN_Y_SPLIT | ffi.GN_AFFINE_F32) if prec else 0
    a.x, a.C1, a.x2 = _ptr(x), C1, _ptr(x2)
    a.gamma, a.beta, a.eps, a.silu = _ptr(gamma), _ptr(beta), eps, int(bool(silu))
    a.y, a.stats, a.stats_doubles = _ptr(out), _ptr(stats), stats.numel()
    _call("idmvton_groupnorm", a, bytes_=(2.0 * x.element_size() + (2 if prec else 1) * out.element_size()) * B * HW * Cc)
    return out


GN_STATS_DOUBLES = 2 * 32 * (2048 + 2 * 64 + 64)


def gn_stats_doubles(B, HW, C, groups):
    return ffi.lib().idmvton_groupnorm_stats_doubles(B, HW, C, groups)


def pack_input(latents, cond, out):
    a = ffi.PackInputArgs()
    B, hw = latents.shape[0], latents.shape[2] * latents.shape[3] if latents.dim() == 4 else latents.shape[2]
    a.dtype, a.B, a.hw, a.cpad = _dt(out), B, hw, out.shape[-1]
    a.latents, a.cond, a.out = _ptr(latents), _ptr(cond), _ptr(out)
    _call("idmvton_pack_input", a)
    return out


def cfg_step(eps_nhwc, latents, noise, coef):
    a = ffi.CfgStepArgs()
    B = latents.shape[0]
    hw = latents.numel() // (B * 4)
    a.dtype, a.B, a.hw, a.ldc = _dt(eps_nhwc), B, hw, eps_nhwc.shape[-1]
    a.eps_nhwc, a.latents, a.noise, a.coef = _ptr(eps_nhwc), _ptr(latents), _ptr(noise), _ptr(coef)
    _call("idmvton_cfg_step", a)
    return latents


def to_nhwc(src_nchw_f32, dtype, cpad=None, scale=1.0, shift=0.0, out=None, split=False):
    B, Cc = src_nchw_f32.shape[:2]
    HW = src_nchw_f32.numel() // (B * Cc)
    cpad = Cc if cpad is None else cpad
    if out is None:
        out = torch.empty((B, HW, 2 * cpad if split else cpad), dtype=dtype, device=src_nchw_f32.device)
    a = ffi.LayoutArgs()
    a.flags = ffi.LAYOUT_SPLIT if split else 0
    a.dtype, a.B, a.C, a.HW, a.cpad, a.to_nhwc = _dt(out), B, Cc, HW, cpad, 1
    a.src, a.dst, a.scale, a.shift = _ptr(src_nchw_f32), _ptr(out), scale, shift
    _call("idmvton_layout", a)
    return out


def to_nchw(src_nhwc, Cc, shape_hw, scale=1.0, shift=0.0, out=None):
    B, HW, cpad = src_nhwc.shape
    if out is None:
        out = torch.empty((B, Cc) + tuple(shape_hw), dtype=torch.float32, device=src_nhwc.device)
    a = ffi.LayoutArgs()
    f32 = src_nhwc.dtype == torch.float32
    a.flags = ffi.LAYOUT_NHWC_F32 if f32 else 0
    a.dtype, a.B, a.C, a.HW, a.cpad, a.to_nhwc = (ffi.BF16 if f32 else _dt(src_nhwc)), B, Cc, HW, cpad, 0
    a.src, a.dst, a.scale, a.shift = _ptr(src_nhwc), _ptr(out), scale, shift
    _call("idmvton_layout", a)
    return out


def vae_sample(moments_nhwc, noise, scale, out=None):
    B, hw, ldm = moments_nhwc.shape
    if out is None:
        out = torch.empty_like(noise)
    a = ffi.VaeSampleArgs()
    a.dtype, a.B, a.hw, a.ldm = _dt(moments_nhwc), B, hw, ldm
    a.moments, a.noise, a.z, a.scale = _ptr(moments_nhwc), _ptr(noise), _ptr(out), scale
    _call("idmvton_vae_sample", a)
    return out


def softmax_rows(x, scale, n_valid=0):
    a = ffi.SoftmaxArgs()
    a.dtype, a.rows, a.n, a.ld = _dt(x), x.shape[0], x.shape[1], x.stride(0)
    a.x, a.scale, a.n_valid = _ptr(x), scale, n_valid
    _call("idmvton_softmax_rows", a)
    return x


def softmax_rows_split(x, scale, dtype, n_valid=0):
    rows, n = x.shape
    out = torch.empty((rows, 2 * n), dtype=dtype, device=x.device)
    a = ffi.SoftmaxArgs()
    a.n_valid = n_valid
    a.dtype, a.rows, a.n, a.ld = _dt(out), rows, n, x.stride(0)
    a.x, a.scale, a.y_split, a.ldy = _ptr(x), scale, _ptr(out), out.stride(0)
    _call("idmvton_softmax_rows", a, bytes_=float(rows * n * (3 * 4 + 2 * out.element_size())))
    return out


def split(x, dtype, mode=ffi.SPLIT_ACT):
    rows, cols = x.shape
    shape = {ffi.SPLIT_ACT: (rows, 2 * cols), ffi.SPLIT_W3: (rows, 3 * cols), ffi.SPLIT_W3T: (cols, 3 * rows)}[mode]
    out = torch.empty(shape, dtype=dtype, device=x.device)
    a = ffi.SplitArgs()
    a.dtype, a.mode, a.rows, a.cols = _dt(out), mode, rows, cols
    a.src, a.lds, a.dst, a.ldd = _ptr(x), x.stride(0), _ptr(out), out.stride(0)
    _call("idmvton_split", a, bytes_=float(rows * cols * 4 + out.numel() * out.element_size()))
    return out


def probe_mfma(which, a, b):
    c = torch.empty((64, 16), dtype=torch.float32, device=a.device)
    rc = ffi.lib().idmvton_probe_mfma(which, C.c_void_p(a.data_ptr()), C.c_void_p(b.data_ptr()),
                                      C.c_void_p(c.data_ptr()), C.c_void_p(_stream()))
    if rc != 0:
        raise RuntimeError(ffi.lib().idmvton_last_error().decode())
    return c


load_tune()
```

### idm-vton_amd/unet.py

```python
import math
import os

import torch

from . import ffi, ops
from .config import UNetConfig, unet_topology
from .weights import conv_weight_nhwc, conv_weight_nhwc_padded, interleave_geglu


def _pad64(c):
    return (c + 63) // 64 * 64


class _Conv:

    def __init__(self, sd, name, cin_pad=None, shortcut=None, pad_out_to=None):
        w = sd[name + ".weight"]
        b = sd[name + ".bias"]
        self.k = w.shape[-1]
        self.cin = w.shape[1]
        self.cin_pad = cin_pad or self.cin
        wk = conv_weight_nhwc_padded(w, self.cin_pad) if self.cin_pad != self.cin else conv_weight_nhwc(w)
        if shortcut is not None:
            ws = sd[shortcut + ".weight"]
            wk = torch.cat([wk, ws.reshape(ws.shape[0], ws.shape[1])], dim=1)
            b = (b.float() + sd[shortcut + ".bias"].float()).to(b.dtype)
        self.cout = w.shape[0]
        if pad_out_to and pad_out_to > self.cout:
            wk = torch.cat([wk, torch.zeros(pad_out_to - self.cout, wk.shape[1], dtype=wk.dtype, device=wk.device)])
            b = torch.cat([b, torch.zeros(pad_out_to - self.cout, dtype=b.dtype, device=b.device)])
        self.w = wk.contiguous()
        self.b = b.contiguous()
        self.n = self.w.shape[0]


class HipUNet:
    def __init__(self, cfg: UNetConfig, state_dict, dtype=torch.bfloat16, device="cuda", stream_f32=False, attn_fp8=False, fuse_xattn=True):
        self.cfg, self.dtype, self.device = cfg, dtype, torch.device(device)
        self.stream_f32 = bool(stream_f32)
        self.attn_fp8 = bool(attn_fp8)
        self.fuse_xattn = bool(fuse_xattn) and os.environ.get("IDMVTON_FUSE_XATTN", "1") != "0"
        self.f8_exp = (2, 2, 2)
        self.f8_fused = os.environ.get("IDMVTON_F8_FUSED", "1") != "0"
        self.topo = unet_topology(cfg)
        sd = {k: v.to(device=self.device, dtype=dtype) for k, v in state_dict.items() if not k.startswith("encoder_hid_proj.")}
        self.sd = sd
        for h, c in zip(cfg.num_attention_heads, cfg.block_out_channels):
            assert c % 64 == 0 and (c // h == 64), "HIP attention kernels are specialised for head_dim 64"
        self.tryon = cfg.mode == "tryon"
        self.ip_scale = 1.0
        self.cin_pad = _pad64(cfg.in_channels)
        self._prep()
        self._gn_stats = torch.empty(ops.GN_STATS_DOUBLES, dtype=torch.float64, device=self.device)
        self._ctx = None

    def _prep(self):
        sd, cfg = self.sd, self.cfg
        self.conv_in = _Conv(sd, "conv_in", cin_pad=self.cin_pad)
        self.res = {}
        self.tf = {}
        temb_w, temb_b, self.temb_slices, off = [], [], {}, 0

        def prep_res(p, cin, cout):
            sc = p + ".conv_shortcut" if cin != cout else None
            self.res[p] = dict(conv1=_Conv(sd, p + ".conv1"), conv2=_Conv(sd, p + ".conv2", shortcut=sc), cin=cin, cout=cout)
            nonlocal off
            temb_w.append(sd[p + ".time_emb_proj.weight"])
            temb_b.append(sd[p + ".time_emb_proj.bias"])
            self.temb_slices[p] = (off, cout)
            off += cout

        def prep_tf(p, ch, n_tf, heads, level):
            blocks = []
            for k in range(n_tf):
                b = f"{p}.transformer_blocks.{k}"
                d = dict(heads=heads)
                d["qkv"] = torch.cat([sd[f"{b}.attn1.to_q.weight"], sd[f"{b}.attn1.to_k.weight"], sd[f"{b}.attn1.to_v.weight"]]).contiguous()
                d["kv_text"] = torch.cat([sd[f"{b}.attn2.to_k.weight"], sd[f"{b}.attn2.to_v.weight"]]).contiguous()
                if self.tryon:
                    d["kv_ip"] = torch.cat([sd[f"{b}.attn2.processor.to_k_ip.weight"], sd[f"{b}.attn2.processor.to_v_ip.weight"]]).contiguous()
                d["ff1_w"], d["ff1_b"] = interleave_geglu(sd[f"{b}.ff.net.0.proj.weight"], sd[f"{b}.ff.net.0.proj.bias"])
                d["p"] = b
                blocks.append(d)
            self.tf[p] = dict(blocks=blocks, ch=ch, heads=heads, level=level)

        level = 0
        for i, blk in enumerate(self.topo["down"]):
            for j, (ci, co) in enumerate(blk["resnets"]):
                prep_res(f"down_blocks.{i}.resnets.{j}", ci, co)
                if blk["attn"]:
                    prep_tf(f"down_blocks.{i}.attentions.{j}", blk["ch"], blk["n_tf"], blk["heads"], level)
            if blk["down"]:
                self.res[f"down_blocks.{i}.downsamplers.0.conv"] = _Conv(sd, f"down_blocks.{i}.downsamplers.0.conv")
                level += 1
        m = self.topo["mid"]
        prep_res("mid_block.resnets.0", m["ch"], m["ch"])
        prep_tf("mid_block.attentions.0", m["ch"], m["n_tf"], m["heads"], level)
        prep_res("mid_block.resnets.1", m["ch"], m["ch"])
        for i, blk in enumerate(self.topo["up"]):
            if self.tryon or blk["attn"]:
                for j, (rin, skip, co) in enumerate(blk["resnets"]):
                    prep_res(f"up_blocks.{i}.resnets.{j}", rin + skip, co)
                    if blk["attn"]:
                        prep_tf(f"up_blocks.{i}.attentions.{j}", blk["ch"], blk["n_tf"], blk["heads"], level)
                if blk["up"]:
                    self.res[f"up_blocks.{i}.upsamplers.0.conv"] = _Conv(sd, f"up_blocks.{i}.upsamplers.0.conv")
            if blk["up"]:
                level -= 1
        self.block_order = [blk for tf in self.tf.values() for blk in tf["blocks"]]
        self.temb_w = torch.cat(temb_w).contiguous()
        self.temb_b = torch.cat(temb_b).contiguous()
        if self.tryon:
            self.conv_out = _Conv(sd, "conv_out", pad_out_to=_pad64(cfg.out_channels) if cfg.out_channels % 4 else None)

    def time_embeddings(self, timesteps, batch, added_cond=None):
        cfg, sd, dt = self.cfg, self.sd, self.dtype
        ts = torch.as_tensor(timesteps, dtype=torch.float32, device=self.device).reshape(-1)
        half = cfg.block_out_channels[0] // 2
        freq = torch.exp(-math.log(10000.0) * torch.arange(half, dtype=torch.float32, device=self.device) / half)
        ang = ts[:, None] * freq[None, :]
        t_emb = torch.cat([torch.cos(ang), torch.sin(ang)], dim=-1).to(dt)
        S = ts.numel()
        mp = max(S, 1)
        e = ops.linear(t_emb.contiguous(), sd["time_embedding.linear_1.weight"], bias=sd["time_embedding.linear_1.bias"])
        e = ops.linear(torch.nn.functional.silu(e.float()).to(dt), sd["time_embedding.linear_2.weight"], bias=sd["time_embedding.linear_2.bias"])
        emb = e[:, None, :].expand(S, batch, -1)
        if cfg.addition_embed_type == "text_time":
            text_embeds, time_ids = added_cond["text_embeds"], added_cond["time_ids"]
            h2 = cfg.addition_time_embed_dim // 2
            f2 = torch.exp(-math.log(10000.0) * torch.arange(h2, dtype=torch.float32, device=self.device) / h2)
            a2 = time_ids.to(self.device).float().flatten()[:, None] * f2[None, :]
            te = torch.cat([torch.cos(a2), torch.sin(a2)], dim=-1).reshape(batch, -1)
            add = torch.cat([text_embeds.to(self.device).float(), te], dim=-1).to(dt).contiguous()
            a = ops.linear(add, sd["add_embedding.linear_1.weight"], bias=sd["add_embedding.linear_1.bias"])
            a = ops.linear(torch.nn.functional.silu(a.float()).to(dt), sd["add_embedding.linear_2.weight"], bias=sd["add_embedding.linear_2.bias"])
            emb = (emb.float() + a.float()[None]).to(dt)
        x = torch.nn.functional.silu(emb.float()).to(dt).reshape(S * batch, -1).contiguous()
        out = ops.linear(x, self.temb_w, bias=self.temb_b)
        return out.reshape(S, batch, -1)

    def encode_context(self, text, ip=None):
        dt, dev = self.dtype, self.device
        B, nt, xd = text.shape
        rt = (nt + 31) // 32 * 32
        tpad = torch.zeros(B, rt, xd, dtype=dt, device=dev)
        tpad[:, :nt] = text.to(dev, dt)
        ctx = dict(B=B, nt=nt, rt=rt, kv={})
        if ip is not None:
            ni = ip.shape[1]
            ri = (ni + 31) // 32 * 32
            ipad = torch.zeros(B, ri, xd, dtype=dt, device=dev)
            ipad[:, :ni] = ip.to(dev, dt)
            ctx.update(ni=ni, ri=ri)
        for p, tf in self.tf.items():
            C = tf["ch"]
            for blk in tf["blocks"]:
                kt = torch.empty(B * rt, C, dtype=dt, device=dev)
                vtt = torch.empty(B, C, rt, dtype=dt, device=dev)
                ops.linear(tpad.reshape(B * rt, xd), blk["kv_text"], out=kt, vt=vtt, vt_n0=C, vt_tokens=rt)
                ent = dict(kt=kt, vtt=vtt)
                if ip is not None:
                    ki = torch.empty(B * ri, C, dtype=dt, device=dev)
                    vti = torch.empty(B, C, ri, dtype=dt, device=dev)
                    ops.linear(ipad.reshape(B * ri, xd), blk["kv_ip"], out=ki, vt=vti, vt_n0=C, vt_tokens=ri)
                    ent.update(ki=ki, vti=vti)
                ctx["kv"][blk["p"]] = ent
        return ctx

    def _gn(self, xa, xb, name, eps, silu):
        sd = self.sd
        return ops.groupnorm(xa, sd[name + ".weight"], sd[name + ".bias"], self.cfg.norm_num_groups, eps, silu,
                             self._gn_stats, x2=xb)

    def _conv3(self, x, cv, B, H, W, stride=1, ups=False, extra_segs=(), out_hw=None, **kw):
        Ho, Wo = (out_hw or (H * 2, W * 2)) if ups else ((H + 2 - 3) // stride + 1, (W + 2 - 3) // stride + 1)
        segs = ops.conv_segs(x, 3, 1, length=cv.cin_pad) + list(extra_segs)
        out = ops.gemm_conv(segs, cv.w, B * Ho * Wo, Ho=Ho, Wo=Wo, Hi=H, Wi=W, stride=stride, ups=ups, bias=cv.b, **kw)
        return out.view(B, Ho * Wo, cv.n), Ho, Wo

    def _resnet(self, p, xa, xb, temb, B, H, W):
        r = self.res[p]
        eps = self.cfg.norm_eps
        g1 = self._gn(xa, xb, p + ".norm1", eps, True)
        off, co = self.temb_slices[p]
        h, _, _ = self._conv3(g1, r["conv1"], B, H, W, rowbias=temb[:, off:off + co], rowbias_ld=temb.stride(0),
                              rows_per_group=H * W)
        g2 = self._gn(h, None, p + ".norm2", eps, True)
        if r["cin"] != r["cout"]:
            extra = [ops.SegSpec(xa, 0, xa.shape[-1])] + ([ops.SegSpec(xb, 0, xb.shape[-1])] if xb is not None else [])
            out, _, _ = self._conv3(g2, r["conv2"], B, H, W, extra_segs=extra)
        else:
            out, _, _ = self._conv3(g2, r["conv2"], B, H, W, res=xa.reshape(B * H * W, -1))
        return out

    def _block(self, blk, hs, B, N, C, ctx, garment, feats_out, stop=None, last=False, nk=None):
        sd, p, heads = self.sd, blk["p"], blk["heads"]
        dt, dev = self.dtype, self.device
        M = B * N
        nk = N if nk is None else nk
        feat = None
        if not self.tryon:
            fb = garment.get("feats_buf") if garment else None
            feat = fb[len(feats_out)][:B].view(M, C) if fb is not None else torch.empty(M, C, dtype=dt, device=dev)
        f8 = self._f8_fused(N)
        eq, ek, ev = self.f8_exp
        f8kw = dict(f8=(2.0 ** ek, 2.0 ** ev)) if f8 else {}
        qk = torch.empty(M, 2 * C, dtype=torch.uint8 if f8 else dt, device=dev)
        vt = torch.empty(B, C, N, dtype=torch.uint8 if f8 else dt, device=dev)
        qcs = ops.QSCALE * (2.0 ** (eq - ek) if f8 else 1.0)
        n1 = ops.layernorm(hs, sd[p + ".norm1.weight"], sd[p + ".norm1.bias"], 1e-5, out2=feat)
        if feat is not None:
            feats_out.append(feat.view(B, N, C))
            if stop is not None and len(feats_out) >= stop:
                return None
        ops.linear(n1, blk["qkv"], out=qk, vt=vt, vt_n0=2 * C, vt_tokens=N, colscale_n=C, colscale=qcs, **f8kw)
        segs = [dict(k=qk[:, C:], vt=vt, nk=nk, ldk=2 * C, ldvt=N, k_rows=N)]
        if self.tryon:
            if garment.get("kv") is not None:
                kg, vtg = garment["kv"][garment["idx"]]
                Bg = vtg.shape[0]
            else:
                g = garment["feats"][garment["idx"]]
                Bg = g.shape[0]
                if g.shape[1] != N:
                    gp = torch.zeros(Bg, N, C, dtype=dt, device=dev)
                    gp[:, :g.shape[1]] = g
                    g = gp
                kg = torch.empty(Bg * N, C, dtype=torch.uint8 if f8 else dt, device=dev)
                vtg = torch.empty(Bg, C, N, dtype=torch.uint8 if f8 else dt, device=dev)
                ops.linear(g.reshape(Bg * N, C), blk["qkv"][C:], out=kg, vt=vtg, vt_n0=C, vt_tokens=N, **f8kw)
            garment["idx"] += 1
            P = garment.get("persons") or Bg
            gseg = dict(k=kg, vt=vtg, nk=nk, ldk=C, ldvt=N, k_rows=N, b0=B - P)
            if Bg < P:
                gseg["nb"] = Bg
            segs.append(gseg)
        att = torch.empty(M, C, dtype=dt, device=dev)
        if self.attn_fp8:
            segs8 = []
            for sg in segs:
                Bs = sg["vt"].shape[0]
                if sg["k"].dtype == torch.uint8:
                    segs8.append(dict(k8=sg["k"], vt8=sg["vt"], nk=nk, ldk=sg["ldk"], ldvt=N, k_rows=N, b0=sg.get("b0", 0), nb=sg.get("nb", 0)))
                    continue
                k8 = ops.quant_f8(sg["k"], 2.0 ** ek)
                vt8 = ops.quant_f8(sg["vt"].reshape(Bs * C, N), 2.0 ** ev, mode=1)
                segs8.append(dict(k8=k8, vt8=vt8, nk=nk, ldk=C, ldvt=vt8.shape[1], k_rows=N, b0=sg.get("b0", 0), nb=sg.get("nb", 0)))
            if f8:
                q8, ldq8 = qk, 2 * C
            else:
                q8, ldq8 = ops.quant_f8(qk[:, :C], 2.0 ** eq), C
            ops.attention_f8(q8, att, segs8, heads, qk_scale_exp=-(eq + ek), v_scale_exp=-ev, B=B, Nq=N, ldq=ldq8, ldo=C)
        else:
            ops.attention(qk, att, segs, heads, B=B, Nq=N, ldq=2 * C, ldo=C, q_prescaled=True)
        f32 = hs.dtype == torch.float32
        hs = ops.linear(att, sd[p + ".attn1.to_out.0.weight"], bias=sd[p + ".attn1.to_out.0.bias"], res=hs, out_f32=f32)
        kv = ctx["kv"][p]
        seg_t = dict(k=kv["kt"], vt=kv["vtt"], nk=ctx["nt"], ldk=C, ldvt=ctx["rt"], k_rows=ctx["rt"])
        xsegs = [seg_t] + ([dict(k=kv["ki"], vt=kv["vti"], nk=ctx["ni"], ldk=C, ldvt=ctx["ri"], k_rows=ctx["ri"])] if self.tryon else [])
        if self.fuse_xattn and N % 32 == 0 and not (C >= 1280 and M >= 8192) and \
                all(sg["nk"] <= (96, 32)[i] and sg["k_rows"] >= (sg["nk"] + 31) // 32 * 32 for i, sg in enumerate(xsegs)):
            if "q2_xw" not in blk:
                blk["q2_xw"] = ops.xattn_q_weight(sd[p + ".attn2.to_q.weight"])
            n2 = ops.layernorm(hs, sd[p + ".norm2.weight"], sd[p + ".norm2.bias"], 1e-5)
            att2 = ops.linear(n2, blk["q2_xw"], xattn=dict(segs=xsegs, tokens=N, ip_scale=self.ip_scale))
        else:
            n2 = ops.layernorm(hs, sd[p + ".norm2.weight"], sd[p + ".norm2.bias"], 1e-5)
            q2 = ops.linear(n2, sd[p + ".attn2.to_q.weight"])
            att2 = torch.empty(M, C, dtype=dt, device=dev)
            if self.tryon:
                ops.attention(q2, att2, xsegs, heads, mode=ffi.ATTN_CROSS, ip_scale=self.ip_scale, B=B, Nq=N, ldq=C, ldo=C)
            else:
                ops.attention(q2, att2, xsegs, heads, B=B, Nq=N, ldq=C, ldo=C)
        hs = ops.linear(att2, sd[p + ".attn2.to_out.0.weight"], bias=sd[p + ".attn2.to_out.0.bias"], res=hs, out_f32=f32)
        n3 = ops.layernorm(hs, sd[p + ".norm3.weight"], sd[p + ".norm3.bias"], 1e-5)
        gg = ops.linear(n3, blk["ff1_w"], bias=blk["ff1_b"], geglu=True)
        hs = ops.linear(gg, sd[p + ".ff.net.2.weight"], bias=sd[p + ".ff.net.2.bias"], res=hs, out_f32=f32 and not last)
        return hs

    def _transformer(self, p, x, B, H, W, ctx, garment, feats_out, stop_after_feats=None):
        sd, tf = self.sd, self.tf[p]
        C, N = tf["ch"], H * W
        Np = ops.round16(N)
        g = self._gn(x, None, p + ".norm", 1e-6, False)
        if Np == N:
            hs = ops.linear(g.reshape(B * N, C), sd[p + ".proj_in.weight"], bias=sd[p + ".proj_in.bias"], out_f32=self.stream_f32)
        else:
            hs = ops.gemm_conv([ops.SegSpec(g, 0, C)], sd[p + ".proj_in.weight"], B * Np, Ho=1, Wo=Np, Hi=1, Wi=N, bias=sd[p + ".proj_in.bias"],
                               out_f32=self.stream_f32)
        for blk in tf["blocks"]:
            hs = self._block(blk, hs, B, Np, C, ctx, garment, feats_out, stop_after_feats, last=blk is tf["blocks"][-1], nk=N)
            if hs is None:
                return None
        if Np == N:
            out = ops.linear(hs, sd[p + ".proj_out.weight"], bias=sd[p + ".proj_out.bias"], res=x.reshape(B * N, C))
        else:
            out = ops.gemm_conv([ops.SegSpec(hs.view(B, Np, C), 0, C)], sd[p + ".proj_out.weight"], B * N, Ho=1, Wo=N, Hi=1, Wi=Np,
                                bias=sd[p + ".proj_out.bias"], res=x.reshape(B * N, C))
        return out.view(B, N, C)

    def feature_tokens(self, h, w):
        lv = [(h, w)]
        for _ in range(len(self.cfg.block_out_channels) - 1):
            lv.append(((lv[-1][0] + 1) // 2, (lv[-1][1] + 1) // 2))
        return [lv[tf["level"]][0] * lv[tf["level"]][1] for tf in self.tf.values() for _ in tf["blocks"]]

    def num_features(self):
        return sum(len(t["blocks"]) for t in self.tf.values())

    def _f8_fused(self, N):
        return self.attn_fp8 and self.f8_fused and N % 64 == 0

    def project_garment_kv(self, feats, out=None):
        assert self.tryon and len(feats) == len(self.block_order)
        res = []
        for i, (blk, g) in enumerate(zip(self.block_order, feats)):
            Bg, N, C = g.shape
            f8 = self._f8_fused(N)
            if out is not None:
                kg, vtg = out[i][0][:Bg * N], out[i][1][:Bg]
            else:
                kg = torch.empty(Bg * N, C, dtype=torch.uint8 if f8 else self.dtype, device=self.device)
                vtg = torch.empty(Bg, C, N, dtype=torch.uint8 if f8 else self.dtype, device=self.device)
            f8kw = dict(f8=(2.0 ** self.f8_exp[1], 2.0 ** self.f8_exp[2])) if f8 else {}
            ops.linear(g.reshape(Bg * N, C), blk["qkv"][C:], out=kg, vt=vtg, vt_n0=C, vt_tokens=N, **f8kw)
            res.append((kg, vtg))
        return res

    def weights_id(self, select=None):
        from .garment_cache import weights_fingerprint
        ids = self.__dict__.setdefault("_weights_ids", {})
        key = getattr(select, "__name__", None) if select is not None else "all"
        if key not in ids:
            ids[key] = weights_fingerprint({k: v for k, v in self.sd.items() if select is None or select(k)})
        return ids[key]

    def forward(self, x, temb, ctx, B, H, W, garment_feats=None, garment_kv=None, feats_buf=None, garment_persons=None):
        topo = self.topo
        garment = dict(feats=garment_feats, kv=garment_kv, feats_buf=feats_buf, idx=0, persons=garment_persons)
        feats = []
        stop = None if self.tryon else self.num_features()
        h, _, _ = self._conv3(x, self.conv_in, B, H, W)
        skips = [(h, H, W)]
        for i, blk in enumerate(topo["down"]):
            for j in range(len(blk["resnets"])):
                h = self._resnet(f"down_blocks.{i}.resnets.{j}", h, None, temb, B, H, W)
                if blk["attn"]:
                    h = self._transformer(f"down_blocks.{i}.attentions.{j}", h, B, H, W, ctx, garment, feats)
                skips.append((h, H, W))
            if blk["down"]:
                h, H, W = self._conv3(h, self.res[f"down_blocks.{i}.downsamplers.0.conv"], B, H, W, stride=2)
                skips.append((h, H, W))
        h = self._resnet("mid_block.resnets.0", h, None, temb, B, H, W)
        h = self._transformer("mid_block.attentions.0", h, B, H, W, ctx, garment, feats)
        h = self._resnet("mid_block.resnets.1", h, None, temb, B, H, W)
        for i, blk in enumerate(topo["up"]):
            if not self.tryon and not blk["attn"]:
                continue
            for j in range(len(blk["resnets"])):
                s, sh, sw = skips.pop()
                assert (sh, sw) == (H, W), "skip / upsample size mismatch"
                h = self._resnet(f"up_blocks.{i}.resnets.{j}", h, s, temb, B, H, W)
                if blk["attn"]:
                    h = self._transformer(f"up_blocks.{i}.attentions.{j}", h, B, H, W, ctx, garment, feats, stop)
                    if h is None:
                        return None, feats
            if blk["up"]:
                tgt = (skips[-1][1], skips[-1][2]) if skips else (2 * H, 2 * W)
                h, H, W = self._conv3(h, self.res[f"up_blocks.{i}.upsamplers.0.conv"], B, H, W, ups=True, out_hw=tgt)
        if not self.tryon:
            return None, feats
        g = self._gn(h, None, "conv_norm_out", self.cfg.norm_eps, True)
        out, _, _ = self._conv3(g, self.conv_out, B, H, W)
        return out, feats
```

### include/idmvton_hip.h

```cpp
#ifndef IDMVTON_HIP_H
#define IDMVTON_HIP_H
#include <stddef.h>
#include <stdint.h>

#ifdef __cplusplus
extern "C" {
#endif

enum { IDMVTON_OK = 0, IDMVTON_E_SHAPE = -1, IDMVTON_E_DTYPE = -2, IDMVTON_E_ALIGN = -3, IDMVTON_E_LAUNCH = -4,
       IDMVTON_E_ARG = -5 };
enum { IDMVTON_F16 = 0, IDMVTON_BF16 = 1, IDMVTON_F32 = 2, IDMVTON_F8E4M3 = 3  };

const char* idmvton_last_error(void);
int idmvton_abi_version(void);
int idmvton_sizeof(const char* struct_name);

#define IDMVTON_MAX_SEG 24
typedef struct {
    const void* ptr;
    uint32_t bytes;
    int32_t pitch;
    int32_t coff;
    int32_t len;
    int32_t dy, dx;
} idmvton_seg;

enum { IDMVTON_EPI_NONE = 0, IDMVTON_EPI_GEGLU = 1, IDMVTON_EPI_GELU = 2 ,
       IDMVTON_EPI_QUICKGELU = 3 ,
       IDMVTON_EPI_XATTN = 4  };
typedef struct {
    int32_t nseg;
    const void* k[2]; int32_t ldk[2]; int32_t k_rows[2];
    const void* vt[2]; int32_t ldvt[2];
    int32_t nk[2];
    int32_t tokens; float ip_scale;
} idmvton_xattn;
enum { IDMVTON_IO_RES_F32 = 1, IDMVTON_IO_OUT_F32 = 2, IDMVTON_IO_BIAS_F32 = 4, IDMVTON_IO_OUT_F8 = 8 };
typedef struct {
    int32_t dtype;
    const void* w; int32_t N; int32_t Ktot;
    int32_t nseg; idmvton_seg seg[IDMVTON_MAX_SEG];
    int32_t M, Ho, Wo, Hi, Wi, stride, ups;
    void* out; int32_t ldo;
    const void* bias;
    const void* rowbias; int32_t rowbias_ld; int32_t rows_per_group;
    const void* res; int32_t ldr;
    int32_t mode;
    void* vt; int32_t vt_n0; int32_t vt_tokens;
    int32_t tile_hint;
    int32_t vt_perm;
    int32_t io_flags;
    const idmvton_xattn* xattn;
    int32_t colscale_n; float colscale;
    float f8_out_scale, f8_vt_scale;
} idmvton_gemm_conv_args;
int idmvton_gemm_conv(const idmvton_gemm_conv_args* a, void* stream);

enum { IDMVTON_ATTN_SELF = 0, IDMVTON_ATTN_CROSS = 1 };
typedef struct {
    int32_t dtype; int32_t mode;
    int32_t B, heads, Nq;
    const void* q; int32_t ldq;
    void* out; int32_t ldo;
    int32_t nseg;
    const void* k[2]; int32_t ldk[2];
    const void* vt[2]; int32_t ldvt[2];
    int32_t nk[2];
    int32_t k_rows[2];
    int32_t seg_b0[2];
    float ip_scale;
    int32_t tune;
    int32_t q_prescaled;
} idmvton_attn_args;
int idmvton_attn_fwd(const idmvton_attn_args* a, void* stream);
int idmvton_attn_fwd_shared(const idmvton_attn_args* a, const int32_t seg_nb[2], void* stream);

typedef struct {
    int32_t out_dtype; int32_t B, heads, Nq;
    const void* q8; int32_t ldq;
    void* out; int32_t ldo;
    int32_t nseg;
    const void* k8[2]; int32_t ldk[2];
    const void* vt8[2]; int32_t ldvt[2];
    int32_t nk[2]; int32_t k_rows[2]; int32_t seg_b0[2];
    int32_t qk_scale_exp; int32_t v_scale_exp;
} idmvton_attn_f8_args;
int idmvton_attn_f8(const idmvton_attn_f8_args* a, void* stream);
int idmvton_attn_f8_shared(const idmvton_attn_f8_args* a, const int32_t seg_nb[2], void* stream);
typedef struct {
    int32_t dtype; int32_t mode; int32_t rows, cols;
    const void* src; int32_t lds;
    void* dst; int32_t ldd;
    float scale;
} idmvton_quant_f8_args;
int idmvton_quant_f8(const idmvton_quant_f8_args* a, void* stream);

typedef struct {
    int32_t dtype; int32_t B, heads, Lq, Lk, d;
    const void* q; int32_t ldq;
    const void* k; int32_t ldk;
    const void* v; int32_t ldv;
    void* out; int32_t ldo;
    float scale; int32_t causal;
} idmvton_attn_small_args;
int idmvton_attn_small(const idmvton_attn_small_args* a, void* stream);

typedef struct {
    int32_t dtype; int32_t rows, C;
    const void* x; int32_t ldx;
    const void* gamma; const void* beta; float eps;
    void* y; int32_t ldy;
    void* y2; int32_t ldy2;
    int32_t x_f32;
} idmvton_layernorm_args;
int idmvton_layernorm(const idmvton_layernorm_args* a, void* stream);

enum { IDMVTON_GN_X_F32 = 1 , IDMVTON_GN_Y_SPLIT = 2 ,
       IDMVTON_GN_AFFINE_F32 = 4  };
typedef struct {
    int32_t dtype; int32_t B, HW, C, groups;
    const void* x; int32_t C1;
    const void* x2;
    const void* gamma; const void* beta; float eps; int32_t silu;
    void* y;
    double* stats; int32_t stats_doubles;
    int32_t flags;
} idmvton_groupnorm_args;
int idmvton_groupnorm(const idmvton_groupnorm_args* a, void* stream);
int idmvton_groupnorm_stats_doubles(int B, int HW, int C, int groups);

typedef struct {
    int32_t dtype; int32_t B, hw, cpad;
    const float* latents; const void* cond; void* out;
} idmvton_pack_input_args;
int idmvton_pack_input(const idmvton_pack_input_args* a, void* stream);

typedef struct {
    int32_t dtype; int32_t B, hw, ldc;
    const void* eps_nhwc; float* latents; const float* noise; const float* coef;
} idmvton_cfg_step_args;
int idmvton_cfg_step(const idmvton_cfg_step_args* a, void* stream);

enum { IDMVTON_LAYOUT_SPLIT = 1 , IDMVTON_LAYOUT_NHWC_F32 = 2  };
typedef struct {
    int32_t dtype; int32_t B, C, HW, cpad; int32_t to_nhwc;
    const void* src; void* dst; float scale; float shift;
    int32_t flags;
} idmvton_layout_args;
int idmvton_layout(const idmvton_layout_args* a, void* stream);

typedef struct {
    int32_t dtype; int32_t B, hw, ldm;
    const void* moments; const float* noise; float* z; float scale;
} idmvton_vae_sample_args;
int idmvton_vae_sample(const idmvton_vae_sample_args* a, void* stream);

typedef struct {
    int32_t dtype; int32_t rows, n, ld;
    void* x; float scale;
    void* y_split; int32_t ldy;
    int32_t n_valid;
} idmvton_softmax_args;
int idmvton_softmax_rows(const idmvton_softmax_args* a, void* stream);

enum { IDMVTON_SPLIT_ACT = 0, IDMVTON_SPLIT_W3 = 1, IDMVTON_SPLIT_W3T = 2 };
typedef struct {
    int32_t dtype; int32_t mode; int32_t rows, cols;
    const float* src; int32_t lds;
    void* dst; int32_t ldd;
} idmvton_split_args;
int idmvton_split(const idmvton_split_args* a, void* stream);

int idmvton_rccl_unique_id(void* id128);
int idmvton_rccl_comm_init(const void* id128, int rank, int world, void** comm_out);
int idmvton_rccl_bcast_arena(void* comm, void* buf, uint64_t bytes, int root, uint64_t chunk_bytes, void* stream);
int idmvton_rccl_comm_destroy(void* comm);

int idmvton_probe_mfma(int which, const void* a, const void* b, float* c, void* stream);

#ifdef __cplusplus
}
#endif
#endif
```

Baseline: 1.599 images/s.

## Fold transformer LayerNorms into the following Linear GEMMs

Folds the LayerNorm gamma into the weights and applies the norm inside the GEMM epilogue. Per-row mean and variance are accumulated from the A fragments already in registers during the K loop, with a two-pass fallback when cancellation is likely. Column sums and shifts then correct the accumulators. This removes the standalone layernorm kernels and their activation round-trips before the qkv, cross-attention q and GEGLU ff1 projections. In exchange it adds dot-product work and a block sync to the GEMM, and changes numerics slightly because the GEMM now consumes un-normalised bf16 inputs.

```diff
diff --git a/idm-vton_amd/csrc/elementwise.hip b/idm-vton_amd/csrc/elementwise.hip
--- a/idm-vton_amd/csrc/elementwise.hip
+++ b/idm-vton_amd/csrc/elementwise.hip
@@ -222,7 +222,7 @@
 #define SZ(n) if (!strcmp(name, #n)) return (int)sizeof(n);
     SZ(idmvton_seg) SZ(idmvton_gemm_conv_args) SZ(idmvton_attn_args) SZ(idmvton_layernorm_args)
     SZ(idmvton_groupnorm_args) SZ(idmvton_pack_input_args) SZ(idmvton_cfg_step_args) SZ(idmvton_layout_args)
-    SZ(idmvton_vae_sample_args) SZ(idmvton_softmax_args) SZ(idmvton_attn_small_args) SZ(idmvton_attn_f8_args) SZ(idmvton_quant_f8_args) SZ(idmvton_split_args) SZ(idmvton_xattn)
+    SZ(idmvton_vae_sample_args) SZ(idmvton_softmax_args) SZ(idmvton_attn_small_args) SZ(idmvton_attn_f8_args) SZ(idmvton_quant_f8_args) SZ(idmvton_split_args) SZ(idmvton_xattn) SZ(idmvton_ln_fold)
 #undef SZ
     return -1;
 }
diff --git a/idm-vton_amd/csrc/gemm_body.cuh b/idm-vton_amd/csrc/gemm_body.cuh
--- a/idm-vton_amd/csrc/gemm_body.cuh
+++ b/idm-vton_amd/csrc/gemm_body.cuh
@@ -6,7 +6,7 @@
 #include "common.cuh"
 #include "gemm_common.cuh"
 
-template <typename T, int BN, int BM, int WN, int WM, int ST, bool V1, bool LIN, bool PF, bool TR, bool XA = false>
+template <typename T, int BN, int BM, int WN, int WM, int ST, bool V1, bool LIN, bool PF, bool TR, bool XA = false, bool LN = false>
 __device__ __forceinline__ void gemm_body(const GemmParams& p, char* smem, const int m0, const int n0) {
     typedef typename VT<T>::v8 v8;
     typedef typename VT<T>::v4 v4;
@@ -19,6 +19,7 @@
     constexpr int WI = (PW_ + NW - 1) / NW, XI = (PX_ + NW - 1) / NW;
     static_assert(BN % 8 == 0 && BM % 8 == 0 && WN * SN == BN && WM * SM == BM && NI * 32 == SN && MI * 32 == SM, "tile / wave-count mismatch");
     static_assert(!UNEVEN || (V1 && ST == 2), "round-robin piece assignment needs the two-stage ring");
+    static_assert(!LN || (V1 && LIN && (WN == 2 || WN == 4) && LN_SCRATCH(WN, BM, BN) <= WBYTES), "LayerNorm fold: Linear ring tiles, statistics scratch inside one weight stage");
     char* sW = smem;
     char* sX = smem + ST * WBYTES;
 
@@ -141,6 +142,15 @@
 
     auto frag_a = [&](const char* bW, int s, int ni) { return *(const v8*)(bW + a_row[ni] + (((2 * s + u) ^ a_swz[ni]) << 4)); };
     auto frag_b = [&](const char* bX, int s, int mi) { return *(const v8*)(bX + b_row[mi] + (((2 * s + u) ^ b_swz[mi]) << 4)); };
+    float ln_s1[MI], ln_s2[MI];
+#pragma unroll
+    for (int mi = 0; mi < MI; ++mi) ln_s1[mi] = ln_s2[mi] = 0.f;
+    constexpr bool LN_SPLIT = LN && NI < 4;
+    auto ln_stat = [&](const v8 (&b)[MI], int s) {
+        if (LN_SPLIT && (s & (WN - 1)) != wn) return;
+#pragma unroll
+        for (int mi = 0; mi < MI; ++mi) ln_accum<T>(b[mi], ln_s1[mi], ln_s2[mi]);
+    };
     auto compute = [&](int buf, bool spread = false, int t_next = 0, int buf_next = 0) {
         const char* bW = sW + buf * WBYTES;
         const char* bX = sX + buf * XBYTES;
@@ -161,6 +171,7 @@
 #pragma unroll
                     for (int mi = 0; mi < MI; ++mi)
                         acc[ni][mi] = TR ? VT<T>::mfma(b[mi], a[ni], acc[ni][mi]) : VT<T>::mfma(a[ni], b[mi], acc[ni][mi]);
+                if constexpr (LN) ln_stat(b, s);
             }
         } else {
             v8 a[2][NI], b[2][MI];
@@ -184,6 +195,7 @@
                     for (int mi = 0; mi < MI; ++mi)
                         acc[ni][mi] = TR ? VT<T>::mfma(b[s & 1][mi], a[s & 1][ni], acc[ni][mi])
                                          : VT<T>::mfma(a[s & 1][ni], b[s & 1][mi], acc[ni][mi]);
+                if constexpr (LN) ln_stat(b[s & 1], s);
                 __builtin_amdgcn_sched_barrier(0);
             }
         }
@@ -224,6 +236,9 @@
         }
     }
 
+    if constexpr (LN) {
+        ln_fold<T, NI, MI, SN, SM, WN, BM, TR, LN_SPLIT>(p, sW + (nt % ST) * WBYTES, acc, ln_s1, ln_s2, m0, n0, wn, wm, lane);
+    }
     if constexpr (XA) {
         v8 xvf[XA_NV];
         xattn_load_v<T>(p.xa, xa_b, xa_h, lane, xvf);
@@ -232,7 +247,7 @@
     gemm_epilogue<T, NI, MI, SN, SM, TR>(p, acc, m0, n0, wn, wm, lane);
 }
 
-template <typename T, int BN, int BM, int WN, int WM, int ST, bool V1, bool LIN, int OCC, bool PFX = false>
+template <typename T, int BN, int BM, int WN, int WM, int ST, bool V1, bool LIN, int OCC, bool PFX = false, bool LN = false>
 __global__ __launch_bounds__(WN * WM * 64, OCC) void gemm_conv_kernel(const GemmParams p) {
     __shared__ __attribute__((aligned(1024))) char smem[ST * (BN + BM) * 128];
     const int wg = xcd_remap(blockIdx.x, p.tiles_m * p.tiles_n);
@@ -248,14 +263,14 @@
     }
     const int m0 = tm * BM, n0 = tn * BN;
     if constexpr (BN == 320) {
-        gemm_body<T, BN, BM, WN, WM, ST, V1, LIN, OCC == 1 || PFX, false>(p, smem, m0, n0);
+        gemm_body<T, BN, BM, WN, WM, ST, V1, LIN, OCC == 1 || PFX, false, false, LN>(p, smem, m0, n0);
     } else {
-        if (p.vt != nullptr && n0 >= p.vt_n0) gemm_body<T, BN, BM, WN, WM, ST, V1, LIN, OCC == 1 || PFX, true>(p, smem, m0, n0);
-        else gemm_body<T, BN, BM, WN, WM, ST, V1, LIN, OCC == 1 || PFX, false>(p, smem, m0, n0);
+        if (p.vt != nullptr && n0 >= p.vt_n0) gemm_body<T, BN, BM, WN, WM, ST, V1, LIN, OCC == 1 || PFX, true, false, LN>(p, smem, m0, n0);
+        else gemm_body<T, BN, BM, WN, WM, ST, V1, LIN, OCC == 1 || PFX, false, false, LN>(p, smem, m0, n0);
     }
 }
 
-template <typename T, int BN, int BM, int WN, int WM, int ST, int OCC>
+template <typename T, int BN, int BM, int WN, int WM, int ST, int OCC, bool LN = false>
 __global__ __launch_bounds__(WN * WM * 64, OCC) void gemm_xattn_kernel(const GemmParams p) {
     __shared__ __attribute__((aligned(1024))) char smem[ST * (BN + BM) * 128];
     const int wg = xcd_remap(blockIdx.x, p.tiles_m * p.tiles_n);
@@ -265,7 +280,7 @@
     const int first = grp * GM;
     const int gsz = p.tiles_m - first < GM ? p.tiles_m - first : GM;
     const int tn = rem / gsz, tm = first + (rem - tn * gsz);
-    gemm_body<T, BN, BM, WN, WM, ST, true, true, OCC == 1, false, true>(p, smem, tm * BM, tn * BN);
+    gemm_body<T, BN, BM, WN, WM, ST, true, true, OCC == 1, false, true, LN>(p, smem, tm * BM, tn * BN);
 }
 
 template <typename T, int BN, int BM, int WN, int WM, int ST, bool V1, int OCC, bool PFX = false>
@@ -274,6 +289,9 @@
     p.gm = V1 ? idmvton_choose_gm(p.tiles_m, p.tiles_n, BM, BN, p.Ktot) : 0;
     const dim3 grid(p.tiles_n * p.tiles_m), block(WN * WM * 64);
     if constexpr (V1) {
+        if constexpr (BN != 320) {
+            if (lin && p.ln_cs) { hipLaunchKernelGGL((gemm_conv_kernel<T, BN, BM, WN, WM, ST, true, true, OCC, PFX, true>), grid, block, 0, st, p); return; }
+        }
         if (lin) { hipLaunchKernelGGL((gemm_conv_kernel<T, BN, BM, WN, WM, ST, true, true, OCC, PFX>), grid, block, 0, st, p); return; }
     }
     hipLaunchKernelGGL((gemm_conv_kernel<T, BN, BM, WN, WM, ST, V1, false, OCC, PFX>), grid, block, 0, st, p);
diff --git a/idm-vton_amd/csrc/gemm_common.cuh b/idm-vton_amd/csrc/gemm_common.cuh
--- a/idm-vton_amd/csrc/gemm_common.cuh
+++ b/idm-vton_amd/csrc/gemm_common.cuh
@@ -19,6 +19,7 @@
     int bias32;
     int out8; float o8_scale, vt8_scale;
     XAttnParams xa;
+    const float* ln_cs; const float* ln_sh; float ln_eps;
 };
 
 int idmvton_choose_gm(int tiles_m, int tiles_n, int bm, int bn, int K);
@@ -31,6 +32,105 @@
         const auto r = __builtin_amdgcn_permlane32_swap(__float_as_uint(c[8 * gp + j]), __float_as_uint(c[8 * gp + 4 + j]), false, false);
         v[j] = __uint_as_float(r[0]);
         v[4 + j] = __uint_as_float(r[1]);
+    }
+}
+
+template <typename T> __device__ __forceinline__ void ln_accum(const typename VT<T>::v8& x, float& s1, float& s2) {
+    typedef __attribute__((ext_vector_type(2))) T v2;
+#pragma unroll
+    for (int i = 0; i < 4; ++i) {
+        v2 q; q[0] = x[2 * i]; q[1] = x[2 * i + 1];
+        v2 one; one[0] = (T)1.0f; one[1] = (T)1.0f;
+        if constexpr (sizeof(T) == 2 && __is_same(T, bf16_t)) {
+            s1 = __builtin_amdgcn_fdot2_f32_bf16(q, one, s1, false);
+            s2 = __builtin_amdgcn_fdot2_f32_bf16(q, q, s2, false);
+        } else {
+            s1 = __builtin_amdgcn_fdot2(q, one, s1, false);
+            s2 = __builtin_amdgcn_fdot2(q, q, s2, false);
+        }
+    }
+}
+
+#define LN_TWO_PASS_T 16.0f
+#define LN_SCRATCH(WN, BM, BN) (((WN) + 1) * (BM) * 8 + (BN) * 8)
+
+template <typename T, int NI, int MI, int SN, int SM, int WN, int BM, bool TR, bool SPLIT>
+__device__ __forceinline__ void ln_fold(const GemmParams& p, char* scr, f32x16 (&acc)[NI][MI], float (&s1)[MI], float (&s2)[MI], const int m0,
+                                        const int n0, const int wn, const int wm, const int lane) {
+    typedef typename VT<T>::v8 v8;
+    const int u = lane >> 5, l31 = lane & 31;
+    float2* part = (float2*)scr;
+    float2* stat = part + WN * BM;
+    constexpr int BN = WN * SN;
+    float* csh = (float*)(stat + BM);
+    for (int i = threadIdx.x; i < 2 * BN; i += WN * (BM / SM) * 64) {
+        const int n = n0 + (i < BN ? i : i - BN);
+        csh[i] = n < p.N ? (i < BN ? p.ln_cs : p.ln_sh)[n] : 0.f;
+    }
+#pragma unroll
+    for (int mi = 0; mi < MI; ++mi) {
+        s1[mi] = xhalf_sum(s1[mi]); s2[mi] = xhalf_sum(s2[mi]);
+        if (SPLIT && u == 0) part[wn * BM + wm * SM + mi * 32 + l31] = make_float2(s1[mi], s2[mi]);
+    }
+    if constexpr (SPLIT) __syncthreads();
+    if (wn == 0 && u == 0) {
+        const float invk = 1.0f / (float)p.Ktot;
+#pragma unroll
+        for (int mi = 0; mi < MI; ++mi) {
+            const int row = wm * SM + mi * 32 + l31;
+            float a = s1[mi], b = s2[mi];
+            if constexpr (SPLIT) {
+                a = b = 0.f;
+#pragma unroll
+                for (int w = 0; w < WN; ++w) { const float2 q = part[w * BM + row]; a += q.x; b += q.y; }
+            }
+            const float mu = a * invk;
+            float var = fmaf(-mu, mu, b * invk);
+            if (var * LN_TWO_PASS_T < mu * mu) {
+                const T* xr = (const T*)p.seg[0].ptr + (size_t)(m0 + row) * p.seg[0].pitch + p.seg[0].coff;
+                float q = 0.f;
+                for (int k = 0; k < p.Ktot; k += 8) {
+                    const v8 x = *(const v8*)(xr + k);
+#pragma unroll
+                    for (int j = 0; j < 8; ++j) { const float d = (float)x[j] - mu; q = fmaf(d, d, q); }
+                }
+                var = q * invk;
+            }
+            stat[row] = make_float2(mu, __builtin_amdgcn_rsqf(fmaxf(var, 0.f) + p.ln_eps));
+        }
+    }
+    __syncthreads();
+    if constexpr (TR) {
+#pragma unroll
+        for (int ni = 0; ni < NI; ++ni) {
+            const float cs = csh[wn * SN + ni * 32 + l31], sh = csh[BN + wn * SN + ni * 32 + l31];
+#pragma unroll
+            for (int mi = 0; mi < MI; ++mi)
+#pragma unroll
+                for (int g = 0; g < 4; ++g) {
+                    const float4* sp = (const float4*)(stat + wm * SM + mi * 32 + 8 * g + 4 * u);
+                    const float4 q0 = sp[0], q1 = sp[1];
+                    const float mu[4] = {q0.x, q0.z, q1.x, q1.z}, rs[4] = {q0.y, q0.w, q1.y, q1.w};
+#pragma unroll
+                    for (int j = 0; j < 4; ++j) acc[ni][mi][4 * g + j] = fmaf(rs[j], fmaf(-mu[j], cs, acc[ni][mi][4 * g + j]), sh);
+                }
+        }
+    } else {
+        float2 st[MI];
+#pragma unroll
+        for (int mi = 0; mi < MI; ++mi) st[mi] = stat[wm * SM + mi * 32 + l31];
+#pragma unroll
+        for (int ni = 0; ni < NI; ++ni)
+#pragma unroll
+            for (int g = 0; g < 4; ++g) {
+                const int c = wn * SN + ni * 32 + 8 * g + 4 * u;
+                const float4 c4 = *(const float4*)(csh + c), h4 = *(const float4*)(csh + BN + c);
+                const float cs[4] = {c4.x, c4.y, c4.z, c4.w}, sh[4] = {h4.x, h4.y, h4.z, h4.w};
+#pragma unroll
+                for (int mi = 0; mi < MI; ++mi)
+#pragma unroll
+                    for (int j = 0; j < 4; ++j) acc[ni][mi][4 * g + j] = fmaf(st[mi].y, fmaf(-st[mi].x, cs[j], acc[ni][mi][4 * g + j]), sh[j]);
+            }
     }
 }
 
diff --git a/idm-vton_amd/csrc/gemm_conv.hip b/idm-vton_amd/csrc/gemm_conv.hip
--- a/idm-vton_amd/csrc/gemm_conv.hip
+++ b/idm-vton_amd/csrc/gemm_conv.hip
@@ -91,8 +91,15 @@
     return IDMVTON_OK;
 }
 
-extern "C" int idmvton_gemm_conv(const idmvton_gemm_conv_args* a, void* stream) {
+static int gemm_conv_impl(const idmvton_gemm_conv_args* a, const idmvton_ln_fold* ln, void* stream) {
     CHECK_ARG(a != nullptr, IDMVTON_E_ARG, "gemm_conv: null args");
+    if (ln) {
+        CHECK_ARG(ln->cs && ln->sh && (((uintptr_t)ln->cs | (uintptr_t)ln->sh) & 15) == 0 && ln->eps > 0.f, IDMVTON_E_ARG,
+                  "gemm_conv_ln: cs / sh (fp32 [N], 16-byte aligned) and eps > 0");
+        CHECK_ARG(a->dtype == IDMVTON_F16 || a->dtype == IDMVTON_BF16, IDMVTON_E_ARG, "gemm_conv_ln: the A operand must be fp16 / bf16 (dtype %d)", a->dtype);
+        CHECK_ARG(a->nseg == 1 && a->Ktot > 0 && a->Ktot % 64 == 0 && a->seg[0].len == a->Ktot, IDMVTON_E_ARG,
+                  "gemm_conv_ln: one K segment with K %% 64 == 0 (nseg=%d K=%d)", a->nseg, a->Ktot);
+    }
     CHECK_ARG(a->dtype == IDMVTON_F16 || a->dtype == IDMVTON_BF16, IDMVTON_E_DTYPE, "gemm_conv: dtype %d", a->dtype);
     CHECK_ARG(a->M > 0 && a->N > 0 && a->Ktot > 0, IDMVTON_E_SHAPE, "gemm_conv: M=%d N=%d K=%d", a->M, a->N, a->Ktot);
     CHECK_ARG(a->Ktot % 64 == 0, IDMVTON_E_SHAPE, "gemm_conv: Ktot=%d must be a multiple of 64", a->Ktot);
@@ -158,6 +165,7 @@
     p.vt = a->vt; p.vt_n0 = a->vt_n0; p.vt_tokens = a->vt_tokens > 0 ? a->vt_tokens : 4; p.vt_perm = a->vt_perm ? 1 : 0;
     p.colscale_n = a->colscale_n; p.colscale = a->colscale;
     p.tiles_m = p.tiles_n = 0; p.gm = 0;
+    p.ln_cs = ln ? ln->cs : nullptr; p.ln_sh = ln ? ln->sh : nullptr; p.ln_eps = ln ? ln->eps : 0.f;
     {
         auto a16 = [](const void* q) { return ((uintptr_t)q & 15) == 0; };
         const int n_out = geglu ? a->N / 2 : a->N;
@@ -212,6 +220,17 @@
         else if (bn == 128 && bm == 128) variant = 6;
         if (a->N > 256 && a->N <= 320 && p.wide && !a->vt && !geglu && !p.out8 && (a->M + 191) / 192 >= 200) { variant = 6; bn = 320; bm = 192; }
     }
+    if (ln) {
+        CHECK_ARG(lin, IDMVTON_E_ARG, "gemm_conv_ln: a plain Linear only (no spatial gather, stride or upsample)");
+        CHECK_ARG(variant != 0 && bn != 320, IDMVTON_E_ARG, "gemm_conv_ln: tile family without the fold (variant %d, %dx%d)", variant, bn, bm & ~15);
+    }
     hipStream_t st = (hipStream_t)stream;
     return launch_gemm(p, a->dtype == IDMVTON_BF16, variant, bn, bm, lin, st);
 }
+
+extern "C" int idmvton_gemm_conv(const idmvton_gemm_conv_args* a, void* stream) { return gemm_conv_impl(a, nullptr, stream); }
+
+extern "C" int idmvton_gemm_conv_ln(const idmvton_gemm_conv_args* a, const idmvton_ln_fold* ln, void* stream) {
+    CHECK_ARG(ln != nullptr, IDMVTON_E_ARG, "gemm_conv_ln: null ln");
+    return gemm_conv_impl(a, ln, stream);
+}
diff --git a/idm-vton_amd/csrc/gemm_lin.hip b/idm-vton_amd/csrc/gemm_lin.hip
--- a/idm-vton_amd/csrc/gemm_lin.hip
+++ b/idm-vton_amd/csrc/gemm_lin.hip
@@ -1,7 +1,7 @@
 #include "gemm_common.cuh"
 #include <type_traits>
 
-template <typename T, int BM, int WN, int WM, int DMA_SPLIT, int WAIT_AT>
+template <typename T, int BM, int WN, int WM, int DMA_SPLIT, int WAIT_AT, bool LN>
 __device__ __forceinline__ void gemm_lin_persistent(const GemmParams& p, char* smem) {
     typedef typename VT<T>::v8 v8;
     constexpr int BN = 256, NW = WN * WM;
@@ -80,10 +80,15 @@
     };
     constexpr int NMF = NI * MI;
     constexpr int NRD = NI + MI;
-    auto pin = [&](int nrd, int nv) {
+    constexpr int NVA = 8 * MI / NMF;
+    constexpr bool LN_SPLIT = LN && NVA > 2;
+    static_assert(!LN_SPLIT || WN == 4, "one k-step per wave of a row block");
+    constexpr bool STAT = LN && !LN_SPLIT;
+    auto pin = [&](int nrd, int nv, bool stat = false) {
 #pragma unroll
         for (int i = 0; i < NMF; ++i) {
             __builtin_amdgcn_sched_group_barrier(0x008, 1, 0);
+            if (stat) __builtin_amdgcn_sched_group_barrier(0x002, NVA, 0);
             if (i < nrd) __builtin_amdgcn_sched_group_barrier(0x100, 1, 0);
             if (i >= NMF - nv) __builtin_amdgcn_sched_group_barrier(0x010, 1, 0);
             if (i < nv - NMF) __builtin_amdgcn_sched_group_barrier(0x010, 1, 0);
@@ -97,6 +102,19 @@
 
     auto run_tile = [&](auto trc) {
         constexpr bool TR = decltype(trc)::value;
+        float ln_s1[MI], ln_s2[MI];
+#pragma unroll
+        for (int mi = 0; mi < MI; ++mi) ln_s1[mi] = ln_s2[mi] = 0.f;
+        auto stat = [&](int set) {
+#pragma unroll
+            for (int mi = 0; mi < MI; ++mi) ln_accum<T>(fb[set][mi], ln_s1[mi], ln_s2[mi]);
+        };
+        auto stat_split = [&](int set, int s) {
+            if constexpr (LN_SPLIT) {
+                if (s == wn) stat(set);
+                __builtin_amdgcn_sched_barrier(0);
+            }
+        };
         auto mfma_range = [&](int set, int i0, int i1) {
 #pragma unroll
             for (int k = i0; k < i1; ++k) {
@@ -124,20 +142,26 @@
                 for (int i = 0; i < PWX; ++i) dma_x(i, nxt, koff);
             }
             mfma_range(0, 0, NMF);
-            pin(NRD, DMA_SPLIT == 0 ? PWW : PWW + PWX);
-            __builtin_amdgcn_sched_barrier(0);
+            if constexpr (STAT) stat(0);
+            pin(NRD, DMA_SPLIT == 0 ? PWW : PWW + PWX, STAT);
+            __builtin_amdgcn_sched_barrier(0);
+            stat_split(0, 0);
             read_all(0, 2, cur);
             if constexpr (DMA_SPLIT == 0) {
 #pragma unroll
                 for (int i = 0; i < PWX; ++i) dma_x(i, nxt, koff);
             }
             mfma_range(1, 0, NMF);
-            pin(NRD, DMA_SPLIT == 0 ? PWX : 0);
-            __builtin_amdgcn_sched_barrier(0);
+            if constexpr (STAT) stat(1);
+            pin(NRD, DMA_SPLIT == 0 ? PWX : 0, STAT);
+            __builtin_amdgcn_sched_barrier(0);
+            stat_split(1, 1);
             read_all(1, 3, cur);
             mfma_range(0, 0, NMF);
-            pin(NRD, 0);
-            __builtin_amdgcn_sched_barrier(0);
+            if constexpr (STAT) stat(0);
+            pin(NRD, 0, STAT);
+            __builtin_amdgcn_sched_barrier(0);
+            stat_split(0, 2);
             mfma_range(1, 0, WAIT_AT);
             __builtin_amdgcn_sched_barrier(0);
             asm volatile("s_waitcnt vmcnt(0) lgkmcnt(0)" ::: "memory");
@@ -146,33 +170,50 @@
             __builtin_amdgcn_sched_barrier(0);
             read_all(0, 0, nxt);
             mfma_range(1, WAIT_AT, NMF);
+            if constexpr (STAT) stat(1);
 #pragma unroll
             for (int i = 0; i < NMF - WAIT_AT; ++i) {
                 __builtin_amdgcn_sched_group_barrier(0x008, 1, 0);
+                if (STAT) __builtin_amdgcn_sched_group_barrier(0x002, (8 * MI + NMF - WAIT_AT - 1) / (NMF - WAIT_AT), 0);
                 if (i < NRD) __builtin_amdgcn_sched_group_barrier(0x100, 1, 0);
                 if (i == NMF - WAIT_AT - 1 && NRD > NMF - WAIT_AT) __builtin_amdgcn_sched_group_barrier(0x100, NRD - (NMF - WAIT_AT), 0);
             }
             __builtin_amdgcn_sched_barrier(0);
+            stat_split(1, 3);
             cur = nxt;
         }
         if (has_next) {
             set_offsets(nm0, nn0);
             dma_first(cur ^ BUF);
         }
-        read_all(1, 1, cur);
-        mfma_range(0, 0, NMF);
-        pin(NRD, 0);
-        __builtin_amdgcn_sched_barrier(0);
-        read_all(0, 2, cur);
-        mfma_range(1, 0, NMF);
-        pin(NRD, 0);
-        __builtin_amdgcn_sched_barrier(0);
-        read_all(1, 3, cur);
-        mfma_range(0, 0, NMF);
-        pin(NRD, 0);
-        __builtin_amdgcn_sched_barrier(0);
-        mfma_range(1, 0, NMF);
+        {
+            read_all(1, 1, cur);
+            mfma_range(0, 0, NMF);
+            if constexpr (STAT) stat(0);
+            pin(NRD, 0, STAT);
+            __builtin_amdgcn_sched_barrier(0);
+            stat_split(0, 0);
+            read_all(0, 2, cur);
+            mfma_range(1, 0, NMF);
+            if constexpr (STAT) stat(1);
+            pin(NRD, 0, STAT);
+            __builtin_amdgcn_sched_barrier(0);
+            stat_split(1, 1);
+            read_all(1, 3, cur);
+            mfma_range(0, 0, NMF);
+            if constexpr (STAT) stat(0);
+            pin(NRD, 0, STAT);
+            __builtin_amdgcn_sched_barrier(0);
+            stat_split(0, 2);
+            mfma_range(1, 0, NMF);
+            if constexpr (STAT) stat(1);
+            stat_split(1, 3);
+        }
         if (has_next) asm volatile("s_waitcnt vmcnt(0)" ::: "memory");
+        if constexpr (LN) {
+            __syncthreads();
+            ln_fold<T, NI, MI, SN, SM, WN, BM, TR, LN_SPLIT>(p, smem + cur, acc, ln_s1, ln_s2, m0, n0, wn, wm, lane);
+        }
         gemm_epilogue<T, NI, MI, SN, SM, TR>(p, acc, m0, n0, wn, wm, lane);
     };
 
@@ -191,10 +232,10 @@
     }
 }
 
-template <typename T, int BM, int WN, int WM, int DMA_SPLIT, int WAIT_AT>
+template <typename T, int BM, int WN, int WM, int DMA_SPLIT, int WAIT_AT, bool LN = false>
 __global__ __launch_bounds__(512, 2) void gemm_lin_kernel(const GemmParams p) {
     __shared__ __attribute__((aligned(1024))) char smem[2 * (256 + BM) * 128];
-    gemm_lin_persistent<T, BM, WN, WM, DMA_SPLIT, WAIT_AT>(p, smem);
+    gemm_lin_persistent<T, BM, WN, WM, DMA_SPLIT, WAIT_AT, LN>(p, smem);
 }
 
 static int persistent_grid(int ntiles, int grid_cap) {
@@ -212,6 +253,12 @@
     GemmParams p = p0;
     p.gm = idmvton_choose_gm(p.tiles_m, p.tiles_n, bm, 256, p.Ktot);
     const dim3 grid(persistent_grid(p.tiles_n * p.tiles_m, grid_cap)), block(512);
+    if (p.ln_cs) {
+        if (bm == 192) hipLaunchKernelGGL((gemm_lin_kernel<T, 192, 4, 2, 0, 2, true>), grid, block, 0, st, p);
+        else if (form == 0) hipLaunchKernelGGL((gemm_lin_kernel<T, 256, 2, 4, 0, 2, true>), grid, block, 0, st, p);
+        else hipLaunchKernelGGL((gemm_lin_kernel<T, 256, 2, 4, 1, 2, true>), grid, block, 0, st, p);
+        return 0;
+    }
     if (bm == 192) hipLaunchKernelGGL((gemm_lin_kernel<T, 192, 4, 2, 0, 2>), grid, block, 0, st, p);
     else if (form == 0) hipLaunchKernelGGL((gemm_lin_kernel<T, 256, 2, 4, 0, 2>), grid, block, 0, st, p);
     else hipLaunchKernelGGL((gemm_lin_kernel<T, 256, 2, 4, 1, 2>), grid, block, 0, st, p);
diff --git a/idm-vton_amd/csrc/gemm_tiles_xattn.hip b/idm-vton_amd/csrc/gemm_tiles_xattn.hip
--- a/idm-vton_amd/csrc/gemm_tiles_xattn.hip
+++ b/idm-vton_amd/csrc/gemm_tiles_xattn.hip
@@ -5,10 +5,22 @@
     GemmParams p = p0;
     p.gm = idmvton_choose_gm(p.tiles_m, p.tiles_n, bm, bn, p.Ktot);
     const dim3 grid(p.tiles_n * p.tiles_m);
-    if (bn == 128 && bm == 128 && w8) hipLaunchKernelGGL((gemm_xattn_kernel<T, 128, 128, 2, 4, 3, 2>), grid, dim3(512), 0, st, p);
-    else if (bn == 128 && bm == 64) hipLaunchKernelGGL((gemm_xattn_kernel<T, 128, 64, 2, 2, 3, 2>), grid, dim3(256), 0, st, p);
-    else if (bn == 128 && bm == 128) hipLaunchKernelGGL((gemm_xattn_kernel<T, 128, 128, 2, 2, 3, 1>), grid, dim3(256), 0, st, p);
-    else if (bn == 128 && bm == 256) hipLaunchKernelGGL((gemm_xattn_kernel<T, 128, 256, 2, 4, 3, 2>), grid, dim3(512), 0, st, p);
+    if (bn == 128 && bm == 128 && w8) {
+        if (p.ln_cs) hipLaunchKernelGGL((gemm_xattn_kernel<T, 128, 128, 2, 4, 3, 2, true>), grid, dim3(512), 0, st, p);
+        else hipLaunchKernelGGL((gemm_xattn_kernel<T, 128, 128, 2, 4, 3, 2>), grid, dim3(512), 0, st, p);
+    }
+    else if (bn == 128 && bm == 64) {
+        if (p.ln_cs) hipLaunchKernelGGL((gemm_xattn_kernel<T, 128, 64, 2, 2, 3, 2, true>), grid, dim3(256), 0, st, p);
+        else hipLaunchKernelGGL((gemm_xattn_kernel<T, 128, 64, 2, 2, 3, 2>), grid, dim3(256), 0, st, p);
+    }
+    else if (bn == 128 && bm == 128) {
+        if (p.ln_cs) hipLaunchKernelGGL((gemm_xattn_kernel<T, 128, 128, 2, 2, 3, 1, true>), grid, dim3(256), 0, st, p);
+        else hipLaunchKernelGGL((gemm_xattn_kernel<T, 128, 128, 2, 2, 3, 1>), grid, dim3(256), 0, st, p);
+    }
+    else if (bn == 128 && bm == 256) {
+        if (p.ln_cs) hipLaunchKernelGGL((gemm_xattn_kernel<T, 128, 256, 2, 4, 3, 2, true>), grid, dim3(512), 0, st, p);
+        else hipLaunchKernelGGL((gemm_xattn_kernel<T, 128, 256, 2, 4, 3, 2>), grid, dim3(512), 0, st, p);
+    }
     else return 1;
     return 0;
 }
diff --git a/idm-vton_amd/ffi.py b/idm-vton_amd/ffi.py
--- a/idm-vton_amd/ffi.py
+++ b/idm-vton_amd/ffi.py
@@ -24,6 +24,10 @@
 class XAttn(C.Structure):
     _fields_ = [("nseg", i32), ("k", vp * 2), ("ldk", i32 * 2), ("k_rows", i32 * 2), ("vt", vp * 2), ("ldvt", i32 * 2), ("nk", i32 * 2),
                 ("tokens", i32), ("ip_scale", f32)]
+
+
+class LnFold(C.Structure):
+    _fields_ = [("cs", vp), ("sh", vp), ("eps", f32)]
 
 
 class GemmConvArgs(C.Structure):
@@ -99,14 +103,14 @@
            "idmvton_pack_input_args": PackInputArgs, "idmvton_cfg_step_args": CfgStepArgs,
            "idmvton_layout_args": LayoutArgs, "idmvton_vae_sample_args": VaeSampleArgs, "idmvton_softmax_args": SoftmaxArgs,
            "idmvton_attn_small_args": AttnSmallArgs, "idmvton_attn_f8_args": AttnF8Args, "idmvton_quant_f8_args": QuantF8Args,
-           "idmvton_split_args": SplitArgs, "idmvton_xattn": XAttn}
+           "idmvton_split_args": SplitArgs, "idmvton_xattn": XAttn, "idmvton_ln_fold": LnFold}
 
 SYMBOLS = ["idmvton_last_error", "idmvton_abi_version", "idmvton_sizeof", "idmvton_gemm_conv", "idmvton_attn_fwd",
            "idmvton_layernorm", "idmvton_groupnorm", "idmvton_pack_input", "idmvton_cfg_step", "idmvton_layout",
            "idmvton_vae_sample", "idmvton_softmax_rows", "idmvton_probe_mfma", "idmvton_groupnorm_stats_doubles",
            "idmvton_attn_small", "idmvton_rccl_unique_id", "idmvton_rccl_comm_init", "idmvton_rccl_bcast_arena",
            "idmvton_rccl_comm_destroy", "idmvton_attn_f8", "idmvton_quant_f8", "idmvton_split", "idmvton_attn_fwd_shared",
-           "idmvton_attn_f8_shared"]
+           "idmvton_attn_f8_shared", "idmvton_gemm_conv_ln"]
 
 _lib = None
 
@@ -145,6 +149,8 @@
     for s in ("idmvton_attn_fwd_shared", "idmvton_attn_f8_shared"):
         getattr(L, s).argtypes = [vp, C.POINTER(i32), vp]
         getattr(L, s).restype = C.c_int
+    L.idmvton_gemm_conv_ln.argtypes = [vp, vp, vp]
+    L.idmvton_gemm_conv_ln.restype = C.c_int
     L.idmvton_probe_mfma.argtypes = [C.c_int, vp, vp, vp, vp]
     L.idmvton_groupnorm_stats_doubles.argtypes = [C.c_int] * 4
     L.idmvton_groupnorm_stats_doubles.restype = C.c_int
@@ -165,6 +171,13 @@
         raise RuntimeError(f"{fn_name} failed ({rc}): {L.idmvton_last_error().decode()}")
 
 
+def call_ln(args, ln, stream):
+    L = lib()
+    rc = L.idmvton_gemm_conv_ln(C.byref(args), C.byref(ln), C.c_void_p(stream))
+    if rc != 0:
+        raise RuntimeError(f"idmvton_gemm_conv_ln failed ({rc}): {L.idmvton_last_error().decode()}")
+
+
 def call_shared(fn_name, args, seg_nb, stream):
     L = lib()
     nb = (i32 * 2)(*seg_nb)
diff --git a/idm-vton_amd/ops.py b/idm-vton_amd/ops.py
--- a/idm-vton_amd/ops.py
+++ b/idm-vton_amd/ops.py
@@ -23,8 +23,13 @@
 PROFILE = None
 
 
-def _call(fn_name, args, flops=0.0, bytes_=0.0, seg_nb=None):
-    launch = (lambda: ffi.call(fn_name, args, _stream())) if seg_nb is None else (lambda: ffi.call_shared(fn_name, args, seg_nb, _stream()))
+def _call(fn_name, args, flops=0.0, bytes_=0.0, seg_nb=None, ln=None):
+    if ln is not None:
+        launch = lambda: ffi.call_ln(args, ln, _stream())
+    elif seg_nb is None:
+        launch = lambda: ffi.call(fn_name, args, _stream())
+    else:
+        launch = lambda: ffi.call_shared(fn_name, args, seg_nb, _stream())
     if PROFILE is None:
         launch()
         return
@@ -83,7 +88,7 @@
 
 def gemm_conv(segs, w, M, *, Ho=1, Wo=None, Hi=1, Wi=None, stride=1, ups=False, out=None, ldo=None, bias=None,
               rowbias=None, rowbias_ld=0, rows_per_group=1, res=None, ldr=None, geglu=False, gelu=False, quick_gelu=False, vt=None,
-              vt_n0=0, vt_tokens=0, vt_perm=True, colscale_n=0, colscale=1.0, tile_hint=0, out_f32=False, xattn=None, f8=None):
+              vt_n0=0, vt_tokens=0, vt_perm=True, colscale_n=0, colscale=1.0, tile_hint=0, out_f32=False, xattn=None, f8=None, ln=None):
     if f8 is not None:
         if res is not None or rowbias is not None or geglu or gelu or quick_gelu or (bias is not None and bias.dtype == torch.float32):
             raise ValueError("gemm_conv(f8=...): no residual / rowbias / activation, and the bias in the storage dtype (not fp32)")
@@ -138,8 +143,15 @@
     a.vt_perm = int(bool(vt_perm)) if vt is not None else 0
     a.colscale_n, a.colscale = colscale_n, colscale
     a.tile_hint = tile_hint if tile_hint else _TUNE["gemm"].get(gemm_key(a), 0)
+    lnf = None
+    if ln is not None:
+        cs, sh = ln["cs"], ln["sh"]
+        if cs.dtype != torch.float32 or sh.dtype != torch.float32 or cs.numel() != N or sh.numel() != N or not (cs.is_contiguous() and sh.is_contiguous()):
+            raise TypeError("gemm_conv(ln=...): cs / sh are contiguous float32 [N] vectors")
+        lnf = ffi.LnFold()
+        lnf.cs, lnf.sh, lnf.eps = _ptr(cs), _ptr(sh), float(ln["eps"])
     if RECORD is not None:
-        RECORD.append(("gemm", gemm_key(a), type(a).from_buffer_copy(a), (segs, w, out, bias, rowbias, res, vt, xa, xattn)))
+        RECORD.append(("gemm", gemm_key(a), type(a).from_buffer_copy(a), (segs, w, out, bias, rowbias, res, vt, xa, xattn, ln)))
     seen, xbytes = set(), 0
     for sg in segs:
         if sg.t.data_ptr() not in seen:
@@ -147,8 +159,26 @@
             xbytes += sg.t.numel() * sg.t.element_size()
     esz = w.element_size()
     obytes = (M * (N // 2 if geglu else N)) * (out.element_size() if out is not None else esz) + (M * N * res.element_size() if res is not None else 0)
-    _call("idmvton_gemm_conv", a, flops=2.0 * M * N * Ktot + xflops, bytes_=float(xbytes + N * Ktot * esz + obytes))
-    return out
+    _call("idmvton_gemm_conv_ln" if lnf is not None else "idmvton_gemm_conv", a, flops=2.0 * M * N * Ktot + xflops,
+          bytes_=float(xbytes + N * Ktot * esz + obytes + (8 * N if lnf is not None else 0)), ln=lnf)
+    return out
+
+
+def fold_layernorm(w, gamma, beta, dtype, perm=None, stats_dtype=torch.float32):
+    w64 = w.double()
+    wp = (w64 * gamma.double()[None, :]).to(dtype)
+    cs = wp.double().sum(dim=1)
+    sh = w64 @ beta.double()
+    if perm is not None:
+        wp, cs, sh = wp.index_select(0, perm), cs.index_select(0, perm), sh.index_select(0, perm)
+    return wp.contiguous(), cs.to(stats_dtype).contiguous(), sh.to(stats_dtype).contiguous()
+
+
+def geglu_order_index(two_inner, device=None):
+    inner = two_inner // 2
+    i = torch.arange(two_inner, device=device)
+    blk, r = i // 64, i % 64
+    return torch.where(r < 32, blk * 32 + r, inner + blk * 32 + (r - 32))
 
 
 def xattn_q_weight(w):
diff --git a/idm-vton_amd/unet.py b/idm-vton_amd/unet.py
--- a/idm-vton_amd/unet.py
+++ b/idm-vton_amd/unet.py
@@ -42,7 +42,9 @@
         self.fuse_xattn = bool(fuse_xattn) and os.environ.get("IDMVTON_FUSE_XATTN", "1") != "0"
         self.f8_exp = (2, 2, 2)
         self.f8_fused = os.environ.get("IDMVTON_F8_FUSED", "1") != "0"
+        self.ln_fold = os.environ.get("IDMVTON_LN_FOLD", "1") != "0"
         self.topo = unet_topology(cfg)
+        self._sd_src = state_dict
         sd = {k: v.to(device=self.device, dtype=dtype) for k, v in state_dict.items() if not k.startswith("encoder_hid_proj.")}
         self.sd = sd
         for h, c in zip(cfg.num_attention_heads, cfg.block_out_channels):
@@ -51,6 +53,7 @@
         self.ip_scale = 1.0
         self.cin_pad = _pad64(cfg.in_channels)
         self._prep()
+        del self._sd_src
         self._gn_stats = torch.empty(ops.GN_STATS_DOUBLES, dtype=torch.float64, device=self.device)
         self._ctx = None
 
@@ -70,16 +73,30 @@
             self.temb_slices[p] = (off, cout)
             off += cout
 
+        def src(k):
+            return self._sd_src[k].to(self.device)
+
+        def fold(w, norm, perm=None):
+            wp, cs, sh = ops.fold_layernorm(w, src(norm + ".weight"), src(norm + ".bias"), self.dtype, perm=perm)
+            return dict(w=wp, ln=dict(cs=cs, sh=sh, eps=1e-5))
+
         def prep_tf(p, ch, n_tf, heads, level):
             blocks = []
             for k in range(n_tf):
                 b = f"{p}.transformer_blocks.{k}"
                 d = dict(heads=heads)
-                d["qkv"] = torch.cat([sd[f"{b}.attn1.to_q.weight"], sd[f"{b}.attn1.to_k.weight"], sd[f"{b}.attn1.to_v.weight"]]).contiguous()
+                if self.tryon:
+                    d["kv_g"] = torch.cat([sd[f"{b}.attn1.to_k.weight"], sd[f"{b}.attn1.to_v.weight"]]).contiguous()
+                    d["qkv_ln"] = fold(torch.cat([src(f"{b}.attn1.to_q.weight"), src(f"{b}.attn1.to_k.weight"), src(f"{b}.attn1.to_v.weight")]), f"{b}.norm1")
+                else:
+                    d["qkv"] = torch.cat([sd[f"{b}.attn1.to_q.weight"], sd[f"{b}.attn1.to_k.weight"], sd[f"{b}.attn1.to_v.weight"]]).contiguous()
+                d["q2_xw_ln"] = fold(src(f"{b}.attn2.to_q.weight"), f"{b}.norm2", perm=ops.key_order_index(ch, self.device))
                 d["kv_text"] = torch.cat([sd[f"{b}.attn2.to_k.weight"], sd[f"{b}.attn2.to_v.weight"]]).contiguous()
                 if self.tryon:
                     d["kv_ip"] = torch.cat([sd[f"{b}.attn2.processor.to_k_ip.weight"], sd[f"{b}.attn2.processor.to_v_ip.weight"]]).contiguous()
-                d["ff1_w"], d["ff1_b"] = interleave_geglu(sd[f"{b}.ff.net.0.proj.weight"], sd[f"{b}.ff.net.0.proj.bias"])
+                w1 = sd[f"{b}.ff.net.0.proj.weight"]
+                d["ff1_b"] = interleave_geglu(w1, sd[f"{b}.ff.net.0.proj.bias"])[1]
+                d["ff1_ln"] = fold(src(f"{b}.ff.net.0.proj.weight"), f"{b}.norm3", perm=ops.geglu_order_index(w1.shape[0], self.device))
                 d["p"] = b
                 blocks.append(d)
             self.tf[p] = dict(blocks=blocks, ch=ch, heads=heads, level=level)
@@ -208,12 +225,16 @@
         qk = torch.empty(M, 2 * C, dtype=torch.uint8 if f8 else dt, device=dev)
         vt = torch.empty(B, C, N, dtype=torch.uint8 if f8 else dt, device=dev)
         qcs = ops.QSCALE * (2.0 ** (eq - ek) if f8 else 1.0)
-        n1 = ops.layernorm(hs, sd[p + ".norm1.weight"], sd[p + ".norm1.bias"], 1e-5, out2=feat)
-        if feat is not None:
-            feats_out.append(feat.view(B, N, C))
-            if stop is not None and len(feats_out) >= stop:
-                return None
-        ops.linear(n1, blk["qkv"], out=qk, vt=vt, vt_n0=2 * C, vt_tokens=N, colscale_n=C, colscale=qcs, **f8kw)
+        fold = self.ln_fold and hs.dtype != torch.float32
+        if self.tryon and fold:
+            ops.linear(hs, blk["qkv_ln"]["w"], ln=blk["qkv_ln"]["ln"], out=qk, vt=vt, vt_n0=2 * C, vt_tokens=N, colscale_n=C, colscale=qcs, **f8kw)
+        else:
+            n1 = ops.layernorm(hs, sd[p + ".norm1.weight"], sd[p + ".norm1.bias"], 1e-5, out2=feat)
+            if feat is not None:
+                feats_out.append(feat.view(B, N, C))
+                if stop is not None and len(feats_out) >= stop:
+                    return None
+            ops.linear(n1, self._unfolded(blk, "qkv"), out=qk, vt=vt, vt_n0=2 * C, vt_tokens=N, colscale_n=C, colscale=qcs, **f8kw)
         segs = [dict(k=qk[:, C:], vt=vt, nk=nk, ldk=2 * C, ldvt=N, k_rows=N)]
         if self.tryon:
             if garment.get("kv") is not None:
@@ -228,7 +249,7 @@
                     g = gp
                 kg = torch.empty(Bg * N, C, dtype=torch.uint8 if f8 else dt, device=dev)
                 vtg = torch.empty(Bg, C, N, dtype=torch.uint8 if f8 else dt, device=dev)
-                ops.linear(g.reshape(Bg * N, C), blk["qkv"][C:], out=kg, vt=vtg, vt_n0=C, vt_tokens=N, **f8kw)
+                ops.linear(g.reshape(Bg * N, C), blk["kv_g"], out=kg, vt=vtg, vt_n0=C, vt_tokens=N, **f8kw)
             garment["idx"] += 1
             P = garment.get("persons") or Bg
             gseg = dict(k=kg, vt=vtg, nk=nk, ldk=C, ldvt=N, k_rows=N, b0=B - P)
@@ -260,23 +281,46 @@
         xsegs = [seg_t] + ([dict(k=kv["ki"], vt=kv["vti"], nk=ctx["ni"], ldk=C, ldvt=ctx["ri"], k_rows=ctx["ri"])] if self.tryon else [])
         if self.fuse_xattn and N % 32 == 0 and not (C >= 1280 and M >= 8192) and \
                 all(sg["nk"] <= (96, 32)[i] and sg["k_rows"] >= (sg["nk"] + 31) // 32 * 32 for i, sg in enumerate(xsegs)):
-            if "q2_xw" not in blk:
-                blk["q2_xw"] = ops.xattn_q_weight(sd[p + ".attn2.to_q.weight"])
-            n2 = ops.layernorm(hs, sd[p + ".norm2.weight"], sd[p + ".norm2.bias"], 1e-5)
-            att2 = ops.linear(n2, blk["q2_xw"], xattn=dict(segs=xsegs, tokens=N, ip_scale=self.ip_scale))
-        else:
-            n2 = ops.layernorm(hs, sd[p + ".norm2.weight"], sd[p + ".norm2.bias"], 1e-5)
-            q2 = ops.linear(n2, sd[p + ".attn2.to_q.weight"])
+            xkw = dict(xattn=dict(segs=xsegs, tokens=N, ip_scale=self.ip_scale))
+            if fold:
+                att2 = ops.linear(hs, blk["q2_xw_ln"]["w"], ln=blk["q2_xw_ln"]["ln"], **xkw)
+            else:
+                if "q2_xw" not in blk:
+                    blk["q2_xw"] = ops.xattn_q_weight(sd[p + ".attn2.to_q.weight"])
+                n2 = ops.layernorm(hs, sd[p + ".norm2.weight"], sd[p + ".norm2.bias"], 1e-5)
+                att2 = ops.linear(n2, blk["q2_xw"], **xkw)
+        else:
+            if fold:
+                if "q2_ln" not in blk:
+                    f, idx = blk["q2_xw_ln"], ops.key_order_index(C, dev)
+                    blk["q2_ln"] = dict(w=f["w"].index_select(0, idx).contiguous(),
+                                        ln=dict(cs=f["ln"]["cs"].index_select(0, idx).contiguous(), sh=f["ln"]["sh"].index_select(0, idx).contiguous(), eps=f["ln"]["eps"]))
+                q2 = ops.linear(hs, blk["q2_ln"]["w"], ln=blk["q2_ln"]["ln"])
+            else:
+                n2 = ops.layernorm(hs, sd[p + ".norm2.weight"], sd[p + ".norm2.bias"], 1e-5)
+                q2 = ops.linear(n2, sd[p + ".attn2.to_q.weight"])
             att2 = torch.empty(M, C, dtype=dt, device=dev)
             if self.tryon:
                 ops.attention(q2, att2, xsegs, heads, mode=ffi.ATTN_CROSS, ip_scale=self.ip_scale, B=B, Nq=N, ldq=C, ldo=C)
             else:
                 ops.attention(q2, att2, xsegs, heads, B=B, Nq=N, ldq=C, ldo=C)
         hs = ops.linear(att2, sd[p + ".attn2.to_out.0.weight"], bias=sd[p + ".attn2.to_out.0.bias"], res=hs, out_f32=f32)
-        n3 = ops.layernorm(hs, sd[p + ".norm3.weight"], sd[p + ".norm3.bias"], 1e-5)
-        gg = ops.linear(n3, blk["ff1_w"], bias=blk["ff1_b"], geglu=True)
+        if fold:
+            gg = ops.linear(hs, blk["ff1_ln"]["w"], ln=blk["ff1_ln"]["ln"], bias=blk["ff1_b"], geglu=True)
+        else:
+            n3 = ops.layernorm(hs, sd[p + ".norm3.weight"], sd[p + ".norm3.bias"], 1e-5)
+            gg = ops.linear(n3, self._unfolded(blk, "ff1_w"), bias=blk["ff1_b"], geglu=True)
         hs = ops.linear(gg, sd[p + ".ff.net.2.weight"], bias=sd[p + ".ff.net.2.bias"], res=hs, out_f32=f32 and not last)
         return hs
+
+    def _unfolded(self, blk, key):
+        if key not in blk:
+            sd, b = self.sd, blk["p"]
+            if key == "qkv":
+                blk[key] = torch.cat([sd[f"{b}.attn1.to_q.weight"], blk["kv_g"]]).contiguous()
+            else:
+                blk[key] = interleave_geglu(sd[f"{b}.ff.net.0.proj.weight"], None)[0]
+        return blk[key]
 
     def _transformer(self, p, x, B, H, W, ctx, garment, feats_out, stop_after_feats=None):
         sd, tf = self.sd, self.tf[p]
@@ -323,7 +367,7 @@
                 kg = torch.empty(Bg * N, C, dtype=torch.uint8 if f8 else self.dtype, device=self.device)
                 vtg = torch.empty(Bg, C, N, dtype=torch.uint8 if f8 else self.dtype, device=self.device)
             f8kw = dict(f8=(2.0 ** self.f8_exp[1], 2.0 ** self.f8_exp[2])) if f8 else {}
-            ops.linear(g.reshape(Bg * N, C), blk["qkv"][C:], out=kg, vt=vtg, vt_n0=C, vt_tokens=N, **f8kw)
+            ops.linear(g.reshape(Bg * N, C), blk["kv_g"], out=kg, vt=vtg, vt_n0=C, vt_tokens=N, **f8kw)
             res.append((kg, vtg))
         return res
 
diff --git a/include/idmvton_hip.h b/include/idmvton_hip.h
--- a/include/idmvton_hip.h
+++ b/include/idmvton_hip.h
@@ -55,6 +55,12 @@
     float f8_out_scale, f8_vt_scale;
 } idmvton_gemm_conv_args;
 int idmvton_gemm_conv(const idmvton_gemm_conv_args* a, void* stream);
+typedef struct {
+    const float* cs;
+    const float* sh;
+    float eps;
+} idmvton_ln_fold;
+int idmvton_gemm_conv_ln(const idmvton_gemm_conv_args* a, const idmvton_ln_fold* ln, void* stream);
 
 enum { IDMVTON_ATTN_SELF = 0, IDMVTON_ATTN_CROSS = 1 };
 typedef struct {
```

Measured after the change: 1.563 images/s. 2.3% lower.
